# Sangluisme/PSgradientSDF

Hardware: AMD Instinct MI355X
Metric: Gauss-Newton iterations/sec (full PS sweep), 256^3 grid x 50 frames (higher is better)
Workload: dtype f32

## Files before the change

### __graft_entry__.py

```python
from __future__ import annotations

import ctypes
import os
import re
import subprocess
import sys

ROOT = os.path.dirname(os.path.abspath(__file__))
if ROOT not in sys.path:
    sys.path.insert(0, ROOT)


def _declared_symbols(header="psgsdf.h"):
    hdr = open(os.path.join(ROOT, "include", header)).read()
    hdr = re.sub(r"/\*.*?\*/", "", hdr, flags=re.S)
    return sorted(set(re.findall(r"\b(psgsdf_[a-z0-9_]+)\s*\(", hdr)) - {"psgsdf_iter_cb"})


def build() -> None:
    csrc = os.path.join(ROOT, "psgradientsdf_amd", "csrc")
    import glob, hashlib
    h = hashlib.sha256()
    for f in sorted(glob.glob(os.path.join(csrc, "*.hip")) + glob.glob(os.path.join(csrc, "*.h")) + glob.glob(os.path.join(ROOT, "psgradientsdf_amd", "host", "*.[ch]pp"))
                    + [os.path.join(csrc, "Makefile"), os.path.join(ROOT, "include", "psgsdf.h"), os.path.join(ROOT, "include", "psgsdf_render.h"),
                       os.path.join(ROOT, "include", "psgsdf_mesh.h"), os.path.join(ROOT, "include", "psgsdf_fit.h")]):
        h.update(os.path.relpath(f, ROOT).encode()); h.update(open(f, "rb").read())
    stamp = os.path.join(csrc, ".build_hash")
    clean = os.environ.get("PSGSDF_BUILD_CLEAN") == "1" or not os.path.exists(stamp) or open(stamp).read() != h.hexdigest() \
        or not os.path.exists(os.path.join(csrc, "libpsgsdf.so")) or not os.path.exists(os.path.join(csrc, "libpsgsdf_dev.so"))
    if clean:
        subprocess.check_call(["make", "-s", "-C", csrc, "clean"])
    import time
    t0 = time.time()
    subprocess.check_call(["make", "-s", "-j16", "-C", csrc])
    print(f"build: build_mode={'from_scratch' if clean else 'up_to_date_by_content_hash'} ({time.time() - t0:.0f} s, source hash {h.hexdigest()[:12]})")
    open(stamp, "w").write(h.hexdigest())
    subprocess.check_call(["make", "-s", "-C", os.path.join(ROOT, "oracle")])
    from psgradientsdf_amd import capi

    for path in (capi.ENGINE_LIB, capi.ENGINE_LIB_DEV):
        lib = ctypes.CDLL(path)
        missing = [s for s in _declared_symbols() + _declared_symbols("psgsdf_render.h") + _declared_symbols("psgsdf_mesh.h") + _declared_symbols("psgsdf_fit.h") if not hasattr(lib, s)]
        if missing:
            raise RuntimeError(f"{os.path.basename(path)} lacks {missing}")


def smoke() -> None:
    import numpy as np
    from psgradientsdf_amd import capi, synth
    from oracle import oracle

    sc = synth.make_scene(N=48, F=6, W=160, H=120, model="SH1")
    st = capi.default_settings(capi.SH1)
    eng = capi.load_engine(sc, sc.K, st, device=0)
    orc = oracle.Oracle(sc, sc.K, st)
    for api in (eng, orc):
        api.load_scene(sc)
        api.init_albedo()
        api.normalize_weights()
    assert eng.info().n_band == orc.info().n_band and eng.info().n_band > 1000
    re_, ro_ = eng.iterate(capi.ALL, 1)[0], orc.iterate(capi.ALL, 1)[0]
    de, do = eng.download_volume(), orc.download_volume()
    band = eng.download_band()
    vs = float(sc.voxel_size)
    err = np.abs(de["dist"][band] - do["dist"][band]).max() / vs
    print(f"smoke: band={len(band)} E_total engine={re_['e_total']:.6f} oracle={ro_['e_total']:.6f} max|d_gpu-d_cpu|/vs={err:.2e}")
    assert abs(re_["e_total"] - ro_["e_total"]) <= 1e-4 * abs(ro_["e_total"])
    assert err < 1e-3
    assert np.abs(eng.download_poses() - orc.download_poses()).max() < 1e-4


if __name__ == "__main__":
    build()
    if len(sys.argv) > 1 and sys.argv[1] == "smoke":
        smoke()
```

### psgradientsdf_amd/capi.py

```python
from __future__ import annotations

import ctypes as C
import os

import numpy as np

ALBEDO, LIGHT, DIST, POSE, ALL = 1, 2, 4, 8, 15
SH1, SH2, LED = 0, 1, 2
L2, CAUCHY, HUBER, TUKEY, TRUNC_L2 = 0, 1, 2, 3, 4
R_DEPTH, R_NORMAL, R_ALBEDO, R_SHADING, R_RENDERED, R_RESIDUAL, R_VOXEL = 1, 2, 4, 8, 16, 32, 64
R_ALL = 127
_R_PLANES = [("depth", R_DEPTH, 1), ("normal", R_NORMAL, 3), ("albedo", R_ALBEDO, 3), ("shading", R_SHADING, 1),
             ("rendered", R_RENDERED, 3), ("residual", R_RESIDUAL, 3), ("voxel", R_VOXEL, 1)]

_HERE = os.path.dirname(os.path.abspath(__file__))
ENGINE_LIB = os.environ.get("PSGSDF_ENGINE_LIB") or os.path.join(_HERE, "csrc", "libpsgsdf.so")
ENGINE_LIB_DEV = os.path.join(_HERE, "csrc", "libpsgsdf_dev.so")


class GridDesc(C.Structure):
    _fields_ = [("dim", C.c_int32 * 3), ("voxel_size", C.c_float), ("shift", C.c_float * 3), ("truncation", C.c_float)]


class Settings(C.Structure):
# ... 440 lines not shown

    def debug_overlap_probe(self, reps=10):
        out = (C.c_double * 4)()
        self._check(self._fn("debug_overlap_probe")(self.ctx, C.c_int(reps), out), "debug_overlap_probe")
        return list(out)

    def debug_normals_cache(self, width, height):
        out = np.empty((9, height, width), np.float32)
        self._check(self._fn("debug_normals_cache")(self.ctx, C.c_int(width), C.c_int(height), out.ctypes.data_as(C.c_void_p)), "debug_normals_cache")
        return out

    def comm_init_sockets(self, peer_fds, rank, n_ranks):
        fds = (C.c_int * n_ranks)(*[int(f) for f in peer_fds])
        self._check(self._fn("comm_init_sockets")(self.ctx, fds, C.c_int(rank), C.c_int(n_ranks)), "comm_init_sockets")

    def comm_allreduce_host(self, values):
        a = np.ascontiguousarray(values, np.float64).copy()
        self._check(self._fn("comm_allreduce_host")(self.ctx, a.ctypes.data_as(C.c_void_p), C.c_int(a.size)), "comm_allreduce_host")
        return a

    def comm_stats(self):
        n = C.c_int64()
        self._check(self._fn("comm_stats")(self.ctx, C.byref(n)), "comm_stats")
        return n.value

    def set_stream(self, stream_ptr):
        self._check(self._fn("set_stream")(self.ctx, C.c_void_p(stream_ptr)), "set_stream")

    def mg_info(self):
        out = (C.c_int32 * 12)()
        self._check(self._fn("mg_info")(self.ctx, out), "mg_info")
        return dict(zip(self._MG_INFO_NAMES, list(out)))

    _MG_INFO_NAMES = ["S", "rows", "row0", "row1", "halo", "F", "rank", "n_ranks", "need_lo", "need_hi", "z0", "z1"]

    def get_tuning(self):
        import json
        f = getattr(self._lib, self._p + "get_tuning"); f.restype = C.c_int
        n = f(self.ctx, None, C.c_size_t(0))
        if n < 0:
            self._check(n, "get_tuning")
        buf = C.create_string_buffer(n + 1)
        f(self.ctx, buf, C.c_size_t(n + 1))
        return json.loads(buf.value.decode())

    def set_profiling(self, on):
        self._check(self._fn("set_profiling")(self.ctx, C.c_int(1 if on else 0)), "set_profiling")

    def watch_kernel(self, name):
        self._check(self._fn("watch_kernel")(self.ctx, name.encode() if name else None), "watch_kernel")

    def reset_kernel_times(self):
        self._check(self._fn("reset_kernel_times")(self.ctx), "reset_kernel_times")

    def kernel_times(self):
        cap = 64
        names = (C.c_char_p * cap)(); ms = (C.c_double * cap)(); n = (C.c_int64 * cap)()
        f = getattr(self._lib, self._p + "kernel_times"); f.restype = C.c_int
        k = f(self.ctx, names, ms, n, C.c_int(cap))
        return {names[i].decode(): (ms[i], n[i]) for i in range(k)}

    def debug_dist_system(self, x=None):
        S = self.info().n_band
        diag = np.empty(S, np.float32); rhs = np.empty(S, np.float32)
        y = np.empty(S, np.float32) if x is not None else None
        xa = np.ascontiguousarray(x, np.float32) if x is not None else None
        self._check(self._fn("debug_dist_system")(self.ctx, diag.ctypes.data_as(C.c_void_p), rhs.ctypes.data_as(C.c_void_p),
                                                   xa.ctypes.data_as(C.c_void_p) if x is not None else None,
                                                   y.ctypes.data_as(C.c_void_p) if x is not None else None), "debug_dist_system")
        return diag, rhs, y

    def debug_time_pcg_pass(self, blocks=0, rows=2, ablate=0, reps=50, stamps=False):
        ms = C.c_double(0)
        st = np.zeros((max(blocks, 1), 8), np.int64) if stamps else None
        self._check(self._fn("debug_time_pcg_pass")(self.ctx, C.c_int(blocks), C.c_int(rows), C.c_int(ablate | (1024 if stamps else 0)), C.c_int(reps), C.byref(ms),
                                                     st.ctypes.data_as(C.c_void_p) if stamps else None), "debug_time_pcg_pass")
        return (ms.value, st) if stamps else ms.value

    def debug_time_pcg_solve(self, passes=16, reps=5):
        ms = C.c_double(0); shape = (C.c_int32 * 2)(); st = (C.c_double * 16)()
        self._check(self._fn("debug_time_pcg_solve")(self.ctx, C.c_int(passes), C.c_int(reps), C.byref(ms), shape, st), "debug_time_pcg_solve")
        return ms.value, (shape[0], shape[1]), [x for x in st]

    def debug_sync_stats(self):
        out = (C.c_int64 * 8)()
        self._check(self._fn("debug_sync_stats")(self.ctx, out), "debug_sync_stats")
        return dict(readbacks_checked=out[0], readbacks_late=out[1], persist_fallbacks=out[2] % 1000000, keyframes_compacted=out[2] // 1000000, speculative_starts=out[3] // 1000000, speculative_undos=out[3] % 1000000,
                    cross_rank_ready=out[4] % 10, halo_pushes=out[4] // 10, cross_rank_solves=out[5], cross_rank_mem_kind=out[6], probe_stale=out[7] // 1000000, probe_timeouts=out[7] % 1000000)

    def debug_rare_rows(self):
        r = C.c_int64(); w = C.c_int64()
        self._check(self._fn("debug_rare_rows")(self.ctx, C.byref(r), C.byref(w)), "debug_rare_rows")
        return r.value, w.value

    def debug_frame_system(self, block):
        i = self.info()
        if block == LIGHT:
            n = i.light_stride; nb = 1 if self._settings.model == LED else i.n_frames
        else:
            n = 6; nb = i.n_frames
        H = np.empty((nb, n, n), np.float64); b = np.empty((nb, n), np.float64)
        self._check(self._fn("debug_frame_system")(self.ctx, C.c_int(block), H.ctypes.data_as(C.c_void_p), b.ctypes.data_as(C.c_void_p)), "debug_frame_system")
        return H, b

    def set_frame_solver(self, mode):
        self._check(self._fn("set_frame_solver")(self.ctx, C.c_int(mode)), "set_frame_solver")

    def frame_solver_stats(self, block):
        it = C.c_int32(); err = C.c_double(); ok = C.c_int32(); ap = C.c_int32()
        self._check(self._fn("get_frame_solver_stats")(self.ctx, C.c_int(block), C.byref(it), C.byref(err), C.byref(ok), C.byref(ap)), "get_frame_solver_stats")
        return {"cg_iters": it.value, "cg_error": err.value, "cg_converged": ok.value, "applied": ap.value}

    def debug_frame_cg(self, H, b, max_it=0):
        H = np.ascontiguousarray(H, np.float32); b = np.ascontiguousarray(b, np.float32)
        nb, n = b.shape
        x = np.empty((nb, n), np.float32); it = C.c_int32(); err = C.c_double(); ok = C.c_int32()
        self._check(self._fn("debug_frame_cg")(self.ctx, C.c_int(nb), C.c_int(n), H.ctypes.data_as(C.c_void_p), b.ctypes.data_as(C.c_void_p), x.ctypes.data_as(C.c_void_p),
                                               C.c_int(max_it), C.byref(it), C.byref(err), C.byref(ok)), "debug_frame_cg")
        return x, it.value, err.value, bool(ok.value)

    def debug_albedo_system(self):
        S = self.info().n_band
        H = np.empty((S, 3), np.float32); b = np.empty((S, 3), np.float32)
        self._check(self._fn("debug_albedo_system")(self.ctx, H.ctypes.data_as(C.c_void_p), b.ctypes.data_as(C.c_void_p)), "debug_albedo_system")
        return H, b


class CommXfer(C.Structure):
    _fields_ = [("ptr_dev", C.c_void_p), ("bytes", C.c_size_t), ("peer", C.c_int)]


ALLREDUCE_FN = C.CFUNCTYPE(C.c_int, C.c_void_p, C.c_void_p, C.c_int, C.c_void_p)
SENDRECV_FN = C.CFUNCTYPE(C.c_int, C.c_void_p, C.POINTER(CommXfer), C.c_int, C.POINTER(CommXfer), C.c_int, C.c_void_p)


class CommOps(C.Structure):
    _fields_ = [("user", C.c_void_p), ("allreduce_f64", ALLREDUCE_FN), ("sendrecv", SENDRECV_FN)]


def comm_unique_id() -> bytes:
    buf = (C.c_uint8 * 128)()
    f = engine_lib().psgsdf_comm_unique_id; f.restype = C.c_int
    rc = f(buf)
    if rc != 0:
        raise PsgsdfError(f"psgsdf_comm_unique_id failed rc={rc} (librccl could not be loaded?)")
    return bytes(buf)


def grid_of(sc) -> GridDesc:
    g = GridDesc()
    g.dim[:] = [int(x) for x in sc.dim]
    g.voxel_size = float(sc.voxel_size)
    g.shift[:] = [float(x) for x in sc.shift]
    g.truncation = float(sc.truncation)
    return g


_engine_lib = {}


def engine_lib(dev: bool = False) -> C.CDLL:
    path = ENGINE_LIB_DEV if dev else ENGINE_LIB
    if path not in _engine_lib:
        if not os.path.exists(path):
            raise PsgsdfError(f"HIP engine {path} is missing: run `python -c 'import __graft_entry__ as g; g.build()'`")
        _engine_lib[path] = C.CDLL(path)
# ... 7 lines not shown
```

### psgradientsdf_amd/csrc/api.hip

```cpp
#include "engine_internal.h"

using namespace psge;

namespace psge {
int host_stage(psgsdf_ctx* c, size_t bytes, void** p) {
    if (c->pin_bytes < bytes) {
        HIPCHK(c, hipStreamSynchronize(c->stream));
        if (c->pin_stage) hipHostFree(c->pin_stage);
        c->pin_stage = nullptr; c->pin_bytes = 0;
        const size_t want = bytes + bytes / 4;
        HIPCHK(c, hipHostMalloc(&c->pin_stage, want, hipHostMallocDefault));
        c->pin_bytes = want;
    }
    *p = c->pin_stage;
    return 0;
}
}

extern "C" {

#ifdef PSGSDF_DEV
const char* psgsdf_version(void) { return "psgsdf-hip gfx950 r5 dev (fault-injection and ablation knobs compiled in: libpsgsdf_dev.so, tests and tools only)"; }
#else
const char* psgsdf_version(void) { return "psgsdf-hip gfx950 r5"; }
#endif

static const char* const kKnobs[] = {
    "PSGSDF_PCG_POLL", "PSGSDF_SPECULATE", "PSGSDF_FOLD_IN_NEXT", "PSGSDF_FUSE_ALBEDO", "PSGSDF_FUSE_PCG_INIT", "PSGSDF_PCG_PERSIST", "PSGSDF_PCG_XCD_LOCAL",
    "PSGSDF_PCG_FUSE_ASM", "PSGSDF_PCG_FUSE_APPLY", "PSGSDF_PCG_PIPELINE", "PSGSDF_PCG_TAGM", "PSGSDF_PCG_PREFETCH", "PSGSDF_PCG_COL16", "PSGSDF_PCG_ROWS", "PSGSDF_PCG_BLOCKS",
    "PSGSDF_FM_SOLVE", "PSGSDF_FRAME_SOLVE", "PSGSDF_FM_ROWS", "PSGSDF_IMG_COMPACT", "PSGSDF_XCD_MAP", "PSGSDF_XCD_STRIPE",
    "PSGSDF_XR", "PSGSDF_XF", "PSGSDF_XS", "PSGSDF_XH", "PSGSDF_XR_MEM", "PSGSDF_XWAIT_LOG2", "PSGSDF_SPECULATE_MR", "PSGSDF_CU_MASK",
    "PSGSDF_WAIT_TIMEOUT_S", "PSGSDF_DESTROY_TIMEOUT_S", "PSGSDF_SOLVE_DUMP"};
static const char* const kDevKnobs[] = {"PSGSDF_PCG_ABLATE", "PSGSDF_FAULT_SOLVE", "PSGSDF_FAULT_HALO", "PSGSDF_MBOX_CHECK"};
const char* psgsdf_last_error(const psgsdf_ctx* c) { return c ? c->err : "null context"; }

int psgsdf_create(const psgsdf_grid_desc* grid, const float K[9], const psgsdf_settings* settings, int device, psgsdf_ctx** out) {
    if (!grid || !K || !settings || !out) return PSGSDF_ERR_ARG;
    if (settings->model < 0 || settings->model > 2) return PSGSDF_ERR_ARG;
    int ndev = 0;
    if (hipGetDeviceCount(&ndev) != hipSuccess || ndev <= 0 || device < 0 || device >= ndev) return PSGSDF_ERR_DEVICE;
    if (hipSetDevice(device) != hipSuccess) return PSGSDF_ERR_DEVICE;
    psgsdf_ctx* c = new psgsdf_ctx();
    c->device = device;
    if (const char* e = getenv("PSGSDF_PCG_POLL")) c->pcg_poll = atoi(e) != 0;
    if (const char* e = getenv("PSGSDF_SPECULATE")) c->speculate = atoi(e) != 0;
    if (const char* e = getenv("PSGSDF_FOLD_IN_NEXT")) c->fold_in_next = atoi(e) != 0;
    if (const char* e = getenv("PSGSDF_FUSE_ALBEDO")) c->fuse_albedo = atoi(e) != 0;
    if (const char* e = getenv("PSGSDF_FUSE_PCG_INIT")) c->fuse_pcg_init = atoi(e) != 0;
    if (const char* e = getenv("PSGSDF_PCG_PERSIST")) c->pcg_persist = atoi(e) != 0;
    if (const char* e = getenv("PSGSDF_PCG_XCD_LOCAL")) c->pcg_xcd_local = atoi(e) != 0;
    if (const char* e = getenv("PSGSDF_AREG_DEVICE")) c->areg_device = atoi(e) != 0;
    if (const char* e = getenv("PSGSDF_PCG_FUSE_ASM")) c->pcg_fuse_asm = atoi(e) != 0;
    if (const char* e = getenv("PSGSDF_PCG_PIPELINE")) c->pcg_pipeline = atoi(e) != 0;
    if (const char* e = getenv("PSGSDF_PCG_TAGM")) { c->pcg_tagm = atoi(e) != 0; c->pcg_tagm_mr = atoi(e) >= 2; }
    if (const char* e = getenv("PSGSDF_PCG_PREFETCH")) c->pcg_prefetch = atoi(e) != 0;
    if (const char* e = getenv("PSGSDF_FM_SOLVE")) { c->fm_solve = atoi(e) != 0; c->fm_solve_led = atoi(e) == 1; }
    if (const char* e = getenv("PSGSDF_FRAME_SOLVE")) c->frame_solve = (!strcmp(e, "eigen") || !strcmp(e, "1")) ? 1 : 0;
    if (const char* e = getenv("PSGSDF_XF")) c->xf_enable = atoi(e) != 0;
    if (const char* e = getenv("PSGSDF_XS")) c->xs_enable = atoi(e) != 0;
    if (const char* e = getenv("PSGSDF_XH")) c->xh_enable = atoi(e) != 0;
    if (const char* e = getenv("PSGSDF_XWAIT_LOG2")) { const int l = atoi(e); if (l >= 8 && l <= 30) c->xwait_spins = 1 << l; }
    if (const char* e = getenv("PSGSDF_IMG_COMPACT")) c->img_compact = atoi(e) != 0;
    if (const char* e = getenv("PSGSDF_SPECULATE_MR")) c->speculate_mr = atoi(e) != 0;
    if (const char* e = getenv("PSGSDF_XCD_MAP")) c->xcd_map = atoi(e);
    if (const char* e = getenv("PSGSDF_XCD_STRIPE")) c->xcd_map = (c->xcd_map & 255) | (atoi(e) << 8);
#ifdef PSGSDF_DEV
    if (const char* e = getenv("PSGSDF_PCG_ABLATE")) c->pcg_ablate = atoi(e) & 7;
    if (const char* e = getenv("PSGSDF_MBOX_CHECK")) c->mbox_check = atoi(e) != 0;
    if (const char* e = getenv("PSGSDF_FAULT_SOLVE")) c->fault_solve = atoi(e);
    if (const char* e = getenv("PSGSDF_FAULT_HALO")) c->fault_halo = atoll(e);
#endif
    for (const char* k : kKnobs) if (const char* e = getenv(k)) c->tuning_env.emplace_back(k, e);
    for (const char* k : kDevKnobs) if (const char* e = getenv(k)) {
#ifdef PSGSDF_DEV
        c->tuning_env.emplace_back(k, e);
#else
        c->tuning_ignored.emplace_back(k, e);
#endif
    }
    if (const char* e = getenv("PSGSDF_PCG_FUSE_APPLY")) c->pcg_fuse_apply = atoi(e) != 0;
    if (hipDeviceGetAttribute(&c->num_cu, hipDeviceAttributeMultiprocessorCount, device) != hipSuccess) c->num_cu = 0;
    c->set = *settings; c->reg_n = settings->reg_weight_n; c->reg_l = settings->reg_weight_l; c->reg_r = settings->reg_weight_rho;
    GridP& g = c->grid;
    for (int a = 0; a < 3; ++a) { g.dim[a] = grid->dim[a]; c->shift[a] = grid->shift[a]; }
    g.nvox = (long long)g.dim[0] * g.dim[1] * g.dim[2]; g.koff = 0;
    for (int a = 0; a < 3; ++a) c->gdim[a] = g.dim[a];
    c->gnvox = g.nvox; c->z0 = c->zlo = 0; c->z1 = c->zhi = g.dim[2];
    g.vs = grid->voxel_size; g.vs_inv = 1.f / g.vs; g.T = grid->truncation;
    for (int a = 0; a < 3; ++a) g.origin[a] = c->shift[a] - (float)(0.5 * (double)g.vs) * (float)g.dim[a];
    c->cam.fx = K[0]; c->cam.fy = K[4]; c->cam.cx = K[2]; c->cam.cy = K[5];
    if (const char* e = getenv("PSGSDF_XR")) c->xr_enable = atoi(e) != 0;
    bool stream_ok;
    if (const char* e = getenv("PSGSDF_CU_MASK")) {
        int lo = 0, hi = 0;
        if (sscanf(e, "%d:%d", &lo, &hi) != 2 || lo < 0 || hi <= lo || hi > c->num_cu) { delete c; return PSGSDF_ERR_ARG; }
        std::vector<uint32_t> mask((size_t)(c->num_cu + 31) / 32, 0u);
        for (int i = lo; i < hi; ++i) mask[i / 32] |= 1u << (i % 32);
        stream_ok = hipExtStreamCreateWithCUMask(&c->stream, (uint32_t)mask.size(), mask.data()) == hipSuccess;
        c->cu_mask_lo = lo; c->cu_mask_hi = hi; c->num_cu = hi - lo;
    } else stream_ok = hipStreamCreate(&c->stream) == hipSuccess;
    bool ok = stream_ok
        && hipMalloc(&c->pcg_sc, sizeof(double) * (16 + 8 * (size_t)kPcgMaxBlocks)) == hipSuccess
        && hipMalloc(&c->pcg_part, sizeof(double) * 14 * kPcgMaxBlocks) == hipSuccess
        && hipMalloc(&c->pcg_gran, sizeof(double) * 2 * kSolveGranPlanes * kSolveMaxBlocksHost) == hipSuccess
        && hipMalloc(&c->mg_scal, sizeof(double) * kMgScal) == hipSuccess && hipMalloc(&c->mg_ext, sizeof(double) * 8) == hipSuccess
        && hipMalloc(&c->d_need, 2 * sizeof(int)) == hipSuccess
        && hipMalloc(&c->d_total, sizeof(int)) == hipSuccess
        && hipMalloc(&c->led_light, sizeof(float) * 3) == hipSuccess
        && hipMalloc(&c->fs_stats, sizeof(double) * 8) == hipSuccess && hipMemset(c->fs_stats, 0, sizeof(double) * 8) == hipSuccess
        && hipEventCreate(&c->ev0) == hipSuccess && hipEventCreate(&c->ev1) == hipSuccess;
    if (!ok) { delete c; return PSGSDF_ERR_DEVICE; }
    *out = c;
    return PSGSDF_OK;
}

void psgsdf_destroy(psgsdf_ctx* c) {
    if (!c) return;
    hipSetDevice(c->device);
    if (c->stream) hipStreamSynchronize(c->stream);
    double qt = 15.0; if (const char* e = getenv("PSGSDF_DESTROY_TIMEOUT_S")) qt = atof(e);
    if (xr_quiesce(c, qt)) {
        c->leak_exported = true;
        fprintf(stderr, "psgsdf: rank %d: a peer did not close its mappings of this rank's exchange memory within %.0f s (failed or still running?): that memory is leaked, not freed\n", c->rank, qt);
    }
    free_dense(c);
    hipFree(c->vis_seq); hipFree(c->frame_idx); hipFree(c->img); hipFree(c->img8); hipFree(c->frames); hipFree(c->frames_undo); hipFree(c->led_light); hipFree(c->fs_stats);
    hipFree(c->band_mem); if (!c->leak_exported) hipFree(c->rec_mem); hipFree(c->obs_mem); hipFree(c->stage);
    hipFree(c->ncache); hipFree(c->ntmp); hipFree(c->nout); hipFree(c->ndepth); hipFree(c->track_part); if (c->track_host) hipHostFree(c->track_host); hipFree(c->acc_frame); hipFree(c->frame_part); hipFree(c->frame_done); hipFree(c->part); hipFree(c->pcg_sc); hipFree(c->pcg_part); hipFree(c->pcg_gran); hipFree(c->d_total);
    for (void* p : c->xo_host) if (p) hipHostFree(p);
    if (c->pin_stage) hipHostFree(c->pin_stage);
    if (c->host_buf) hipHostFree(c->host_buf);
    if (c->mbox) hipHostFree(c->mbox);
    if (c->ev0) hipEventDestroy(c->ev0); if (c->ev1) hipEventDestroy(c->ev1);
    for (auto& pr : c->watch_pool) { hipEventDestroy(pr.first); hipEventDestroy(pr.second); }
    if (!c->leak_exported) { hipFree(c->xr); hipFree(c->hx_mem); }
    hipFree(c->xf_table); hipFree(c->vm_order);
    comm_destroy(c);
    hipFree(c->areg_mem); hipFree(c->mg_scal); hipFree(c->mg_ext); hipFree(c->mbox_shadow); hipFree(c->d_need);
    if (c->stream && c->own_stream) hipStreamDestroy(c->stream);
    delete c;
}

static double count_plane(const psgsdf_ctx* c, const float* d, const uint64_t* v, int wpv) {
    const long long plane = (long long)c->gdim[0] * c->gdim[1];
    const float lim = (float)(sqrt(3.0) * (double)c->grid.vs);
    long long m = 0;
    for (long long i = 0; i < plane; ++i) { if (!(fabsf(d[i]) <= lim)) continue; bool seen = false; for (int w = 0; w < wpv && !seen; ++w) seen = v[(size_t)i * wpv + w] != 0; m += seen; }
    return (double)m;
}
static int cut_slabs(psgsdf_ctx* c, std::vector<double>& cnt, int* z0, int* z1) {
    const int nz = c->gdim[2], n = c->n_ranks;
    if (nz < n) return fail(c, PSGSDF_ERR_UNSUPPORTED, "%d z-planes cannot be cut into %d slabs", nz, n);
    if (n > 1) {
        double* d_cnt = nullptr;
        HIPCHK(c, hipMalloc(&d_cnt, sizeof(double) * nz));
        int rc = 0;
        if (hipMemcpyAsync(d_cnt, cnt.data(), sizeof(double) * nz, hipMemcpyHostToDevice, c->stream) != hipSuccess) rc = fail(c, PSGSDF_ERR_DEVICE, "slab histogram upload");
        if (!rc) rc = comm_allreduce(c, d_cnt, nz);
        if (!rc && (hipMemcpyAsync(cnt.data(), d_cnt, sizeof(double) * nz, hipMemcpyDeviceToHost, c->stream) != hipSuccess || hipStreamSynchronize(c->stream) != hipSuccess)) rc = fail(c, PSGSDF_ERR_DEVICE, "slab histogram download");
        hipFree(d_cnt);
        if (rc) return rc;
    }
    double total = 0; for (double x : cnt) total += x;
    if (total <= 0) return fail(c, PSGSDF_ERR_UNSUPPORTED, "the volume has no band candidates to partition");
    std::vector<int> cut(n + 1, 0); cut[n] = nz;
    double run = 0; int r = 1;
    for (int k = 0; k < nz && r < n; ++k) { run += cnt[k]; while (r < n && run >= total * r / n) { cut[r] = k + 1; ++r; } }
    for (int q = 1; q < n; ++q) cut[q] = std::max(cut[q], cut[q - 1] + 1);
    for (int q = n - 1; q >= 1; --q) cut[q] = std::min(cut[q], cut[q + 1] - 1);
    *z0 = cut[c->rank]; *z1 = cut[c->rank + 1];
    return 0;
}
static int choose_slab(psgsdf_ctx* c, const float* dist, const uint64_t* vis_words, int wpv, int* z0, int* z1) {
    const int nz = c->gdim[2], n = c->n_ranks;
    const long long plane = (long long)c->gdim[0] * c->gdim[1];
    std::vector<double> cnt(nz, 0.0);
    for (int k = c->rank; k < nz; k += n) cnt[k] = count_plane(c, dist + (size_t)k * plane, vis_words + (size_t)k * plane * wpv, wpv);
    return cut_slabs(c, cnt, z0, z1);
}

static int upload_planes(psgsdf_ctx* c, int z0, int z1, size_t src_n, size_t src_off, const float* dist, const float* grad_xyz, const float* weight, const float* rgb, const uint64_t* vis_words, int words_per_voxel) {
    { int rc = set_local_grid(c, z0, z1); if (rc) return rc; }
    const long long n = c->grid.nvox;
    free_dense(c);
    if (c->vis_seq) { hipFree(c->vis_seq); c->vis_seq = nullptr; }
    int rc = alloc_dense(c, c->dense, n, 0, true); if (rc) return rc;
    HIPCHK(c, hipMalloc(&c->vis_seq, sizeof(uint64_t) * n * words_per_voxel));
    c->wpv_seq = words_per_voxel;
    HIPCHK(c, hipMemcpyAsync(c->dense.dist, dist + src_off, sizeof(float) * n, hipMemcpyHostToDevice, c->stream));
    for (int a = 0; a < 3; ++a) {
        HIPCHK(c, hipMemcpyAsync(c->dense.g[a], grad_xyz + (size_t)a * src_n + src_off, sizeof(float) * n, hipMemcpyHostToDevice, c->stream));
        HIPCHK(c, hipMemcpyAsync(c->dense.rho[a], rgb + (size_t)a * src_n + src_off, sizeof(float) * n, hipMemcpyHostToDevice, c->stream));
    }
    HIPCHK(c, hipMemcpyAsync(c->dense.weight, weight + src_off, sizeof(float) * n, hipMemcpyHostToDevice, c->stream));
    HIPCHK(c, hipMemcpyAsync(c->vis_seq, vis_words + src_off * words_per_voxel, sizeof(uint64_t) * n * words_per_voxel, hipMemcpyHostToDevice, c->stream));
    HIPCHK(c, hipStreamSynchronize(c->stream));
    c->have_volume = true; c->inited = false;
    return PSGSDF_OK;
}

int psgsdf_upload_volume(psgsdf_ctx* c, const float* dist, const float* grad_xyz, const float* weight, const float* rgb, const uint64_t* vis_words, int words_per_voxel) {
    if (!c || !dist || !grad_xyz || !weight || !rgb || !vis_words || words_per_voxel < 1) return fail(c, PSGSDF_ERR_ARG, "upload_volume: null argument");
    HIPCHK(c, hipSetDevice(c->device));
    int z0 = 0, z1 = c->gdim[2];
    if (c->n_ranks > 1) { int rc = choose_slab(c, dist, vis_words, words_per_voxel, &z0, &z1); if (rc) return rc; }
    const int zlo = std::max(0, z0 - 1);
    return upload_planes(c, z0, z1, (size_t)c->gnvox, (size_t)zlo * c->gdim[0] * c->gdim[1], dist, grad_xyz, weight, rgb, vis_words, words_per_voxel);
}

int psgsdf_slab_plane_count(psgsdf_ctx* c, const float* dist_plane, const uint64_t* vis_plane, int words_per_voxel, double* count) {
    if (!c || !dist_plane || !vis_plane || !count || words_per_voxel < 1) return fail(c, PSGSDF_ERR_ARG, "slab_plane_count: null argument");
// ... 432 lines not shown
```

### psgradientsdf_amd/csrc/api_debug.hip

```cpp
#include "engine_internal.h"

using namespace psge;

extern "C" {
int psgsdf_set_profiling(psgsdf_ctx* c, int enabled) { if (!c) return PSGSDF_ERR_ARG; c->profiling = enabled != 0; return PSGSDF_OK; }
int psgsdf_reset_kernel_times(psgsdf_ctx* c) { if (!c) return PSGSDF_ERR_ARG; c->ktimes.clear(); c->watch_used = 0; return PSGSDF_OK; }
int psgsdf_watch_kernel(psgsdf_ctx* c, const char* name) {
    if (!c) return PSGSDF_ERR_ARG;
    hipStreamSynchronize(c->stream);
    std::string w = name ? name : ""; int every = 1;
    const size_t sl = w.find('/');
    if (sl != std::string::npos) { every = std::max(1, atoi(w.c_str() + sl + 1)); w.resize(sl); }
    c->watch = w; c->watch_every = every; c->watch_seen = 0; c->watch_used = 0;
    return PSGSDF_OK;
}
int psgsdf_kernel_times(psgsdf_ctx* c, const char** names, double* ms, int64_t* launches, int cap) {
    if (!c) return 0;
    if (c->watch_used) {
        hipStreamSynchronize(c->stream);
        KTime& k = c->ktimes[c->watch];
        for (size_t i = 0; i < c->watch_used; ++i) { float t = 0; if (hipEventElapsedTime(&t, c->watch_pool[i].first, c->watch_pool[i].second) == hipSuccess) { k.ms += t; k.n += 1; } }
        c->watch_used = 0;
    }
    int n = 0;
    for (auto& kv : c->ktimes) { if (n >= cap) break; names[n] = kv.first.c_str(); ms[n] = kv.second.ms; launches[n] = kv.second.n; ++n; }
    return n;
}

int psgsdf_debug_dist_system(psgsdf_ctx* c, float* diag, float* rhs, const float* x, float* y) {
    if (!c || !c->inited) return fail(c, PSGSDF_ERR_STATE, "init first");
    HIPCHK(c, hipSetDevice(c->device));
    SweepArgs a = make_args(c, c->reg_l != 0.f);
    launch_sweep_dist(a, c->stream);
    launch_assemble(a, c->stream);
    const int S = c->band.S;
    if (diag) HIPCHK(c, hipMemcpyAsync(diag, c->band.H, sizeof(float) * S, hipMemcpyDeviceToHost, c->stream));
    if (rhs) HIPCHK(c, hipMemcpyAsync(rhs, c->band.rhs, sizeof(float) * S, hipMemcpyDeviceToHost, c->stream));
    if (x && y) {
        HIPCHK(c, hipMemcpyAsync(c->band.x, x, sizeof(float) * S, hipMemcpyHostToDevice, c->stream));
        launch_matvec(a, c->band.x, c->band.t, c->stream);
        HIPCHK(c, hipMemcpyAsync(y, c->band.t, sizeof(float) * S, hipMemcpyDeviceToHost, c->stream));
    }
    HIPCHK(c, hipStreamSynchronize(c->stream));
    return PSGSDF_OK;
}

int psgsdf_debug_time_pcg_pass(psgsdf_ctx* c, int blocks, int rows, int ablate, int reps, double* avg_ms, long long* stamps) {
    if (!c || !c->inited || !avg_ms) return fail(c, PSGSDF_ERR_STATE, "init first");
    HIPCHK(c, hipSetDevice(c->device));
    SweepArgs a = make_args(c, c->reg_l != 0.f);
    launch_sweep_dist(a, c->stream);
    launch_assemble(a, c->stream);
    int G, rdef; cgf_shape(band_blocks(c), &G, &rdef);
    if (blocks > 0) G = std::min(blocks, kCgfMaxBlocks);
    if (rows <= 0) rows = rdef;
    launch_cgf_init(a, c->pcg_sc, c->pcg_part, G, c->stream);
    hipEvent_t e0, e1; HIPCHK(c, hipEventCreate(&e0)); HIPCHK(c, hipEventCreate(&e1));
    for (int q = 0; q < 3; ++q) launch_cgf_pass(a, c->pcg_sc, c->pcg_part, G, rows, q, 1 << 30, c->mbox_dev, c->stream, ablate | 16);
    HIPCHK(c, hipEventRecord(e0, c->stream));
    for (int q = 0; q < reps; ++q) launch_cgf_pass(a, c->pcg_sc, c->pcg_part, G, rows, 3 + q, 1 << 30, c->mbox_dev, c->stream, ablate | 16);
    HIPCHK(c, hipEventRecord(e1, c->stream));
    HIPCHK(c, hipStreamSynchronize(c->stream));
    float ms = 0; HIPCHK(c, hipEventElapsedTime(&ms, e0, e1));
    hipEventDestroy(e0); hipEventDestroy(e1);
    *avg_ms = (double)ms / reps;
    if (stamps) {
        HIPCHK(c, hipMemcpy(stamps, c->pcg_sc + 16, sizeof(long long) * 8 * G, hipMemcpyDeviceToHost));
    }
    return PSGSDF_OK;
}

int psgsdf_debug_time_pcg_solve(psgsdf_ctx* c, int passes, int reps, double* ms_per_launch, int32_t* shape, double* stamps ) {
    if (!c || !c->inited || !ms_per_launch || !shape || (passes < 1 && passes != -7) || reps < 1) return fail(c, PSGSDF_ERR_STATE, "init first");
    HIPCHK(c, hipSetDevice(c->device));
    int G = 0, rows = 0;
    if (!cgf_solve_shape(c, &G, &rows)) return fail(c, PSGSDF_ERR_UNSUPPORTED, "the persistent solve does not apply to this context");
    shape[0] = G; shape[1] = rows;
    SweepArgs a = make_args(c, c->reg_l != 0.f);
    a.pcg_fuse_init = 1; a.pcg_init_blocks = band_blocks(c); a.pcg_gran = c->pcg_gran; a.pcg_gran_n = 2 * kSolveGranPlanes * kSolveMaxBlocksHost; a.pcg_asm = c->pcg_fuse_asm ? 1 : 0;
    hipEvent_t e0, e1; HIPCHK(c, hipEventCreate(&e0)); HIPCHK(c, hipEventCreate(&e1));
    float total = 0;
    for (int r = 0; r < reps + 1; ++r) {
        launch_sweep_dist(a, c->stream);
// ... 76 lines not shown
    if (!c) return PSGSDF_ERR_ARG;
    if (mode != 0 && mode != 1) return fail(c, PSGSDF_ERR_ARG, "frame solver mode %d (0 = LDL^T per frame, 1 = the reference's global float Jacobi-PCG)", mode);
    c->frame_solve = mode;
    return PSGSDF_OK;
}
int psgsdf_get_frame_solver_stats(psgsdf_ctx* c, int block, int32_t* iterations, double* error, int32_t* converged, int32_t* applied) {
    if (!c) return PSGSDF_ERR_ARG;
    if (block != PSGSDF_LIGHT && block != PSGSDF_POSE) return fail(c, PSGSDF_ERR_ARG, "block must be LIGHT or POSE");
    HIPCHK(c, hipSetDevice(c->device));
    const int kind = block == PSGSDF_POSE ? 1 : 0;
    psgsdf_step_stats st; memset(&st, 0, sizeof(st));
    if (int rc = read_frame_solver_stats(c, kind, &st)) return rc;
    if (iterations) *iterations = st.cg_iters;
    if (error) *error = st.cg_error;
    if (converged) *converged = st.cg_converged;
    if (applied) *applied = st.applied;
    return PSGSDF_OK;
}
int psgsdf_debug_frame_cg(psgsdf_ctx* c, int nb, int n, const float* H, const float* b, float* x, int max_it, int32_t* iterations, double* error, int32_t* converged) {
    if (!c || !H || !b || !x || nb <= 0) return fail(c, PSGSDF_ERR_ARG, "null argument");
    if ((n != 3 && n != 4 && n != 6 && n != 9) || (long long)nb * n > 2048) return fail(c, PSGSDF_ERR_UNSUPPORTED, "block size %d x %d blocks", n, nb);
    HIPCHK(c, hipSetDevice(c->device));
    float *dH = nullptr, *db = nullptr, *dx = nullptr; double* ds = nullptr;
    const size_t nH = (size_t)nb * n * n, nv = (size_t)nb * n;
    int rc = PSGSDF_OK;
    if (hipMalloc(&dH, sizeof(float) * nH) != hipSuccess || hipMalloc(&db, sizeof(float) * nv) != hipSuccess || hipMalloc(&dx, sizeof(float) * nv) != hipSuccess || hipMalloc(&ds, sizeof(double) * 4) != hipSuccess)
        rc = fail(c, PSGSDF_ERR_DEVICE, "out of device memory");
    double st[4] = {0, 0, 0, 0};
    if (!rc && (hipMemcpy(dH, H, sizeof(float) * nH, hipMemcpyHostToDevice) != hipSuccess || hipMemcpy(db, b, sizeof(float) * nv, hipMemcpyHostToDevice) != hipSuccess)) rc = fail(c, PSGSDF_ERR_DEVICE, "upload failed");
    if (!rc && launch_frames_eigen_raw(nb, n, dH, db, dx, ds, max_it, c->stream)) rc = fail(c, PSGSDF_ERR_UNSUPPORTED, "shape");
    if (!rc && (hipStreamSynchronize(c->stream) != hipSuccess || hipMemcpy(x, dx, sizeof(float) * nv, hipMemcpyDeviceToHost) != hipSuccess || hipMemcpy(st, ds, sizeof(st), hipMemcpyDeviceToHost) != hipSuccess))
        rc = fail(c, PSGSDF_ERR_DEVICE, "%s", hipGetErrorString(hipGetLastError()));
    hipFree(dH); hipFree(db); hipFree(dx); hipFree(ds);
    if (rc) return rc;
    if (iterations) *iterations = (int32_t)st[0];
    if (error) *error = st[1];
    if (converged) *converged = (int32_t)st[2];
    return PSGSDF_OK;
}
int psgsdf_debug_frame_system(psgsdf_ctx* c, int block, double* H, double* b) {
    if (!c || !c->inited || !H || !b) return fail(c, PSGSDF_ERR_STATE, "init first");
    HIPCHK(c, hipSetDevice(c->device));
    SweepArgs a = make_args(c, 0);
    const bool led = c->set.model == PSGSDF_LED;
    int n, nb, nh;
    int launched = 0;
    if (block == PSGSDF_LIGHT) { launched = launch_sweep_light(a, c->stream); n = led ? 3 : (c->set.model == PSGSDF_SH2 ? 9 : 4); nb = led ? 1 : c->F; nh = led ? 3 : n * (n + 1) / 2; }
    else if (block == PSGSDF_POSE) { launched = launch_sweep_pose(a, c->stream); n = 6; nb = c->F; nh = 21; }
    else return fail(c, PSGSDF_ERR_ARG, "block must be LIGHT or POSE");
    if (!launched) HIPCHK(c, hipMemsetAsync(c->acc_frame, 0, sizeof(double) * c->acc_frame_n, c->stream));
    std::vector<double> acc(c->acc_frame_n);
    HIPCHK(c, hipMemcpyAsync(acc.data(), c->acc_frame, sizeof(double) * c->acc_frame_n, hipMemcpyDeviceToHost, c->stream));
    HIPCHK(c, hipStreamSynchronize(c->stream));
    if (led && block == PSGSDF_LIGHT) {
        for (int i = 0; i < 9; ++i) H[i] = 0;
        for (int i = 0; i < 3; ++i) { b[i] = 0; for (int f = 0; f < c->F; ++f) { H[i * 3 + i] += acc[(size_t)f * kFrameRow + i]; b[i] += acc[(size_t)f * kFrameRow + 3 + i]; } }
        return PSGSDF_OK;
    }
    for (int k = 0; k < nb; ++k) {
        const double* A = acc.data() + (size_t)k * kFrameRow;
        double* Hk = H + (size_t)k * n * n; double* bk = b + (size_t)k * n;
        for (int i = 0; i < n * n; ++i) Hk[i] = 0;
        int q = 0;
        for (int i = 0; i < n; ++i) for (int j = i; j < n; ++j) { Hk[i * n + j] = A[q]; Hk[j * n + i] = A[q]; ++q; }
        for (int i = 0; i < n; ++i) bk[i] = A[nh + i];
    }
    return PSGSDF_OK;
}

int psgsdf_debug_albedo_system(psgsdf_ctx* c, float* H, float* b) {
    if (!c || !c->inited || !H || !b) return fail(c, PSGSDF_ERR_STATE, "init first");
    HIPCHK(c, hipSetDevice(c->device));
    SweepArgs a = make_args(c, 0);
    launch_sweep_albedo(a, c->stream);
    const int S = c->band.S, Sp = c->band.Spad;
    std::vector<float> h(3 * (size_t)Sp), bb(3 * (size_t)Sp);
    HIPCHK(c, hipMemcpyAsync(h.data(), c->band.aH, sizeof(float) * 3 * Sp, hipMemcpyDeviceToHost, c->stream));
    HIPCHK(c, hipMemcpyAsync(bb.data(), c->band.ab, sizeof(float) * 3 * Sp, hipMemcpyDeviceToHost, c->stream));
    HIPCHK(c, hipStreamSynchronize(c->stream));
    for (int j = 0; j < S; ++j) for (int ch = 0; ch < 3; ++ch) { H[3 * j + ch] = h[(size_t)ch * Sp + j]; b[3 * j + ch] = bb[(size_t)ch * Sp + j]; }
    return PSGSDF_OK;
}

int psgsdf_debug_sync_stats(psgsdf_ctx* c, int64_t out[8]) {
    if (!c || !out) return PSGSDF_ERR_ARG;
    out[0] = c->mbox_checked; out[1] = c->mbox_late; out[2] = c->persist_fallbacks + (c->img_compacted ? 1000000LL : 0); out[3] = c->spec_windows * 1000000LL + c->spec_undos;
    out[4] = (c->xr_ready ? 1 : 0) + 10 * c->n_halo_pushes; out[5] = c->xr_solves; out[6] = c->xr_mem_kind; out[7] = c->xr_probe_stale * 1000000LL + c->xr_probe_timeouts;
    return PSGSDF_OK;
}

int psgsdf_get_tuning(psgsdf_ctx* c, char* json, size_t cap) {
    if (!c) return PSGSDF_ERR_ARG;
    std::string o = "{\"build\": \"";
    o += psgsdf_version(); o += "\", \"env\": {";
    auto esc = [](const std::string& v) { std::string r; for (char ch : v) { if (ch == '"' || ch == '\\') r += '\\'; if ((unsigned char)ch >= 0x20) r += ch; } return r; };
    bool first = true;
    for (auto& kv : c->tuning_env) { o += (first ? "\"" : ", \"") + kv.first + "\": \"" + esc(kv.second) + "\""; first = false; }
    o += "}, \"ignored_dev_only\": {"; first = true;
    for (auto& kv : c->tuning_ignored) { o += (first ? "\"" : ", \"") + kv.first + "\": \"" + esc(kv.second) + "\""; first = false; }
    o += "}, \"effective\": {";
    char buf[1024];
    snprintf(buf, sizeof(buf), "\"pcg_poll\": %d, \"speculate\": %d, \"speculate_mr\": %d, \"fold_in_next\": %d, \"fuse_albedo\": %d, \"fuse_pcg_init\": %d, \"pcg_persist\": %d, \"pcg_pipeline\": %d, \"pcg_tagm\": %d, "
             "\"pcg_prefetch\": %d, \"pcg_fuse_asm\": %d, \"pcg_fuse_apply\": %d, \"pcg_xcd_local\": %d, \"fm_solve\": %d, \"fm_solve_led\": %d, \"frame_solve\": \"%s\", \"img_compact\": %d, \"xcd_map\": %d, "
             "\"xr\": %d, \"xf\": %d, \"xs\": %d, \"xh\": %d, \"xr_mem_kind\": %d, \"xwait_log2\": %d, \"cu_mask\": [%d, %d], \"mbox_check\": %d, \"pcg_ablate\": %d, \"fault_solve\": %d, \"fault_halo\": %lld",
             (int)c->pcg_poll, (int)c->speculate, (int)c->speculate_mr, (int)c->fold_in_next, (int)c->fuse_albedo, (int)c->fuse_pcg_init, (int)c->pcg_persist, (int)c->pcg_pipeline, (c->pcg_pipeline && c->pcg_tagm) ? (c->n_ranks > 1 ? (c->pcg_tagm_mr ? 2 : 0) : 1) : 0,
             (int)c->pcg_prefetch, (int)c->pcg_fuse_asm, (int)c->pcg_fuse_apply, (int)c->pcg_xcd_local, (int)c->fm_solve, (int)c->fm_solve_led, c->frame_solve == 1 ? "eigen" : "ldlt", (int)c->img_compact, c->xcd_map,
             (int)c->xr_enable, (int)c->xf_enable, (int)c->xs_enable, (int)c->xh_enable, c->xr_mem_kind, (int)lround(log2((double)c->xwait_spins)), c->cu_mask_lo, c->cu_mask_hi,
             (int)c->mbox_check, c->pcg_ablate, c->fault_solve, c->fault_halo);
    o += buf; o += "}";
    if (c->n_ranks > 1) {
        snprintf(buf, sizeof(buf), ", \"xr_probe\": {\"rank\": %d, \"n_ranks\": %d, \"kind_chosen\": %d, \"stale_mappings\": %lld, \"fine_grained\": {\"tried\": %lld, \"stale_records_from_lower\": %lld, \"expired_waits_lower\": %lld, \"expired_waits_upper\": %lld}, "
                 "\"uncached\": {\"tried\": %lld, \"stale_records_from_lower\": %lld, \"expired_waits_lower\": %lld, \"expired_waits_upper\": %lld}}",
                 c->rank, c->n_ranks, c->xr_mem_kind, c->xr_stale_maps, c->xr_probe_local[1][3], c->xr_probe_local[1][0], c->xr_probe_local[1][1], c->xr_probe_local[1][2],
                 c->xr_probe_local[2][3], c->xr_probe_local[2][0], c->xr_probe_local[2][1], c->xr_probe_local[2][2]);
        o += buf;
    }
    o += "}";
    if (json && cap) { const size_t n = std::min(cap - 1, o.size()); memcpy(json, o.data(), n); json[n] = 0; }
    return (int)o.size();
}

}
```

### psgradientsdf_amd/csrc/engine.h

```cpp
#pragma once
#include <hip/hip_runtime.h>
#include <stdint.h>

namespace psg {

constexpr int kBlock = 256;
constexpr int kMaxFramesLds = 640;
constexpr int kNQ = 19;
constexpr int kNQCommon = 13;
constexpr int kMaxBasis = 9;

struct FrameP {
    float R[9];
    float t[3];
    float l[9];
    float pad[3];
};

struct Cam { float fx, fy, cx, cy; int W, H; };

struct GridP {
    int dim[3];
    long long nvox;
    float vs, vs_inv;
// ... 22 lines not shown
    float4* vp[3];
    float* aH; float* ab;
    float* blk;
    float* H;
    int* hx;
    float* rhs; float* x; float* t;
    float4* rec[2];
    int* obs_ptr;
    int* obs_rows;
    int obs_max;
    long long obs_ptr_total;
};

struct Accum {
    double* frame;
    double* part;
    int PB;
    double* fpart;
    int fcap;
    int* fdone;
};
constexpr int kFrameRow = 64;
constexpr int kPcgMaxBlocks = 2048;
constexpr int kCgfMaxBlocks = 768;

enum { SC_ENERGY = 0, SC_NOBS = 1, SC_EN = 2, SC_EL = 3, SC_ACCEPT = 4, SC_AUX0 = 5, SC_AUX1 = 6, SC_AUX2 = 7, SC_COUNT = 8 };

struct AlbedoReg {
    int* anb;
    int* back;
    float* anrho;
    float* J;
    float* res;
    float* rhs; float* diag; float* diag0; float* x; float* r; float* p; float* q; float* t;
    double* cgs;
    float weight;
};

struct XfTable;
struct FoldReq { int n; int id[4]; int nblk; double* out; unsigned long long key; const XfTable* xf; long long xf_epoch; };

struct ImgSrc {
    const float* f32;
    const unsigned* u8; float scale;
    bool idx32;
};

struct SweepArgs {
    Band b;
    const FrameP* frames;
    ImgSrc im;
    int F;
    Cam cam;
    GridP grid;
    Robust rob;
    Accum acc;
    int model;
    int quirks;
    float reg_n, reg_l;
    int normal_reg, laplacian_reg;
    float damping;
    int row0, row1;
    FoldReq fold;
    AlbedoReg ar;
    double* pcg_part; double* pcg_fs;
    int pcg_asm;
    unsigned pcg_epoch;
    int pcg_pipe;
    int pcg_xcd_local;
    int pcg_apply;
    double* pcg_gran; int pcg_gran_n;
    int pcg_fuse_init;
    int pcg_init_blocks;
    int fuse_apply;
    const int* vm_order;
    float* fm_led_light;
    const XfTable* xf;
    long long xf_epoch;
    int xcd_map;
    int fm_solve;
    FrameP* fm_frames; float* fm_undo; double* fm_e_out; unsigned long long fm_e_key;
    const double* gate;
    const double* ext;
};

constexpr int kXrMaxRanks = 32;
constexpr int kXrPeerTags = 64;
constexpr int kXrRankGran = 0, kXrPtag = 2 * 8 * kXrMaxRanks, kXrAbort = kXrPtag + 2 * 3 * kXrPeerTags, kXrDoubles = kXrAbort + 8;
constexpr int kXrLate = kXrAbort + 1;
constexpr int kXrNonce = kXrAbort + 7;
struct XrArgs {
    int rank, n_ranks;
    double* region[kXrMaxRanks];
    float4* lo_rec[2]; float4* hi_rec[2];
    float4* lo_base[2];
    int give_lo, give_hi;
    int wait_lo, wait_hi;
    int need_lo, need_hi;
    unsigned epoch;
};
struct XfTable {
    int n_ranks, rank, F, spin_max;
    long long pay, flg;
    long long spay, sflg;
    double* region[32];
};
constexpr int kHxWords = 16;
constexpr unsigned kXrEpochMask = 0x3fffu;

constexpr int kTryPackFlags = 2048;
void launch_normals_cache(int W, int H, int r, double fx_inv, double fy_inv, double cx, double cy, double* work , float* out , hipStream_t s);
void launch_try_pack_f32(const float* rgb, unsigned* rgba, size_t npix, size_t stride, float scale, int* fail , hipStream_t s);
void launch_pack_rgb8(const uint8_t* rgb, unsigned* rgba, size_t npix, hipStream_t s);
void launch_select_vis(const uint64_t* vis_seq, int wpv_seq, uint64_t* vis_key, int KW, const int* frame_idx, int F, long long nvox, hipStream_t s);
void launch_band_flags(const float* dist, const uint64_t* vis_key, int KW, float vs, long long nvox, int* flags, hipStream_t s);
void launch_band_scan(int* flags_inout_rowof, long long nvox, int* block_sums, int* d_total, hipStream_t s);
struct DenseView { float* dist; float* g[3]; float* weight; float* rho[3]; uint64_t* vis; int KW; int* row_of; };
void launch_band_fill(const DenseView& d, const GridP& grid, Band b, int* d_reach, hipStream_t s);
void launch_band_scatter(const DenseView& d, Band b, hipStream_t s);
void launch_derive(const SweepArgs& a, int update_grad, hipStream_t s);
constexpr int kObsChunk = 2048;
void launch_obs_count(const Band& b, int F, int row0, int row1, int* counts, hipStream_t s);
void launch_block_work(const Band& b, int row0, int row1, int* work, hipStream_t s);
void launch_obs_fill(const Band& b, int F, int row0, int row1, const int* offsets, hipStream_t s);
void launch_lower_bound(const int* lin, int S, int target, int* out, hipStream_t s);
struct SlotList { int n; int id[8]; };
void launch_sum_parts(const double* part, int PB, int nblk, const SlotList& slots, double* out, unsigned long long key, hipStream_t s, const XfTable* xf = nullptr, long long xf_epoch = 0);
void launch_frame_cols(const double* frame, int F, int col, double* out, unsigned long long key, hipStream_t s);
void launch_zero_f64(double* p, int n, hipStream_t s);
struct CopySegs { int n; unsigned off[16]; unsigned len[16]; unsigned long long key[16]; };
void launch_copy_segs(const double* src, double* dst, const CopySegs& segs, hipStream_t s);
void launch_marker(double* p, double v, hipStream_t s);
void launch_init_albedo(const SweepArgs& a, hipStream_t s);
void launch_led_light_init(const SweepArgs& a, hipStream_t s);
void launch_energy(const SweepArgs& a, hipStream_t s);
void launch_sweep_albedo(const SweepArgs& a, hipStream_t s);
void launch_apply_albedo(const SweepArgs& a, hipStream_t s);
void launch_restore_albedo(const SweepArgs& a, hipStream_t s);
int launch_sweep_light(const SweepArgs& a, hipStream_t s);
int launch_sweep_pose(const SweepArgs& a, hipStream_t s);
void launch_solve_light(const SweepArgs& a, FrameP* frames, float* led_light, double* e_out, unsigned long long e_key, float* undo, hipStream_t s);
void launch_restore_light(int F, FrameP* frames, float* led_light, const float* undo, hipStream_t s);
void launch_solve_pose(const SweepArgs& a, FrameP* frames, double* e_out, unsigned long long e_key, hipStream_t s);
bool frames_eigen_fits(int model, int F);
void launch_frames_eigen_light(const SweepArgs& a, FrameP* frames, float* led_light, double* e_out, unsigned long long e_key, float* undo, double* stats, hipStream_t s);
void launch_frames_eigen_pose(const SweepArgs& a, FrameP* frames, double* e_out, unsigned long long e_key, double* stats, hipStream_t s);
int launch_frames_eigen_raw(int nb, int n, const float* H, const float* b, float* x, double* stats, int max_it, hipStream_t s);
void launch_sweep_dist(const SweepArgs& a, hipStream_t s);
void launch_assemble(const SweepArgs& a, hipStream_t s);
void launch_cgf_init(const SweepArgs& a, double* fs, double* part, int G, hipStream_t s);
void launch_cgf_pass(const SweepArgs& a, double* fs, double* part, int G, int rows, int k, int kmax, double* mb, hipStream_t s, int ablate = 0);
void launch_cgf_sum(double* part, int G, int k, double* out, hipStream_t s);
constexpr int kSolveGranPlanes = 8;
constexpr int kSolveThreadsHost = 512, kSolveMaxBlocksHost = 256, kSolveMaxRowsHost = 4, kSolveMbSlots = 24;
int cgf_solve_max_blocks(int rows);
void launch_cgf_solve(const SweepArgs& a, double* fs, double* gran, int G, int rows_per_wg, int kmax, double* mb, unsigned long long mb_key, int force_passes, hipStream_t s, const XrArgs* xr = nullptr);
void launch_areg_tables(const DenseView& d, const GridP& g, const SweepArgs& a, hipStream_t s);
void launch_areg_build(const SweepArgs& a, hipStream_t s);
void launch_areg_system(const SweepArgs& a, hipStream_t s);
void launch_areg_jx(const SweepArgs& a, const float* p, float* t, hipStream_t s);
void launch_areg_jt(const SweepArgs& a, const float* p, const float* t, float* q, hipStream_t s);
void launch_areg_cg_init(const SweepArgs& a, hipStream_t s);
void launch_areg_cg_iteration(const SweepArgs& a, int i, int nblk, float thr, hipStream_t s);
void launch_areg_cg_update(const SweepArgs& a, float alpha, hipStream_t s);
void launch_areg_cg_dir(const SweepArgs& a, float beta, hipStream_t s);
void launch_apply_albedo_delta(const SweepArgs& a, const float* delta, hipStream_t s);
void launch_matvec(const SweepArgs& a, const float* x, float* y, hipStream_t s);
void launch_apply_dist(const SweepArgs& a, hipStream_t s);
void launch_upsample(const DenseView& src, const DenseView& dst, const GridP& g_old, hipStream_t s);
void launch_fill_f32(float* p, float v, long long n, hipStream_t s);
void launch_normals(const float* depth, const float* cache, int W, int H, int r, double* tmp, float* out, hipStream_t s);
void launch_track(const DenseView& d, const GridP& g, const Cam& cam, const FrameP& fp, const float* depth, float z_min, float z_max, double* part, int nblk, int gdimz, int zown0, int zown1, hipStream_t s);
void launch_integrate(const DenseView& d, uint64_t* vis_seq, int wpv_seq, const GridP& g, const Cam& cam, const FrameP& fp,
                      const float* rgb, const float* depth, const float* normals, int counter, float z_min, float z_max, hipStream_t s);

constexpr int kRenderBrick = 8;
constexpr int kRenderTile = 8;
constexpr int kRenderStats = 9;
enum { RP_DEPTH = 0, RP_NORMAL, RP_ALBEDO, RP_SHADING, RP_RENDERED, RP_RESIDUAL, RP_VOXEL, RP_COUNT };
enum { RF_DEPTH = 0, RF_NORMAL = 1, RF_ALBEDO = 4, RF_SHADING = 7, RF_RENDERED = 8, RF_VOXEL = 11, RF_OFF_BAND = 12, RF_COUNT = 13 };
struct RenderArgs {
    DenseView d;
    const float4* vp[3];
    GridP grid;
    const FrameP* frames;
    ImgSrc im; int img_w, img_h;
    Robust rob;
    const unsigned char* bricks;
    const int* bbox;
    int nb[3];
    Cam cam;
    int frame;
    int light_frame;
    FrameP pose;
    int tiles_x, tiles_y;
    float* planes[RP_COUNT];
    double* part;
    int zr[2];
    int slab;
    int f0;
    double* mask;
    unsigned char* mine;
    double* rec;
    long long rec_px;
    int rf[RF_COUNT];
    int n_rf;
};
void launch_render_bricks(const DenseView& d, const GridP& g, float thr, int z0, int z1, unsigned char* bricks, int* bbox, double* marks, hipStream_t s);
void launch_render_box(const double* marks, const int* nb, unsigned char* bricks, int* bbox, hipStream_t s);
void launch_render(const RenderArgs& a, int model, hipStream_t s);
void launch_render_report(const RenderArgs& a, int model, int F, hipStream_t s);
void launch_render_fold(const double* part, int tiles, int F, double* out , hipStream_t s);
void launch_render_ranks(const RenderArgs& a, int model, bool report, int chunk, hipStream_t s);
void launch_render_keep(const RenderArgs& a, hipStream_t s);
void launch_render_composite(const RenderArgs& a, bool report, int chunk, hipStream_t s);

struct WMeshGrid {
    const float* dist; const float* weight; const float* g[3]; const float* rho[3];
    const float* hg[3]; const float* hrho[3];
    int nx, ny, zlo, zh;
    int lo[3], d[3];
    int zc0;
    long long nown;
    float voxel[3], origin[3];
};
void launch_wmesh_mark(const WMeshGrid& g, long long ncell, int* cnt, int* flag, hipStream_t s);
void launch_wmesh_or(int* dst, const int* src, long long n, hipStream_t s);
void launch_wmesh_faces(const WMeshGrid& g, long long ncell, const int* offs, int n_faces, const int* num, int first, const int* num_up, int first_up, int* faces, hipStream_t s);
void launch_wmesh_verts(const WMeshGrid& g, const int* num, int n_verts, float* xyz, float* nrm, unsigned char* rgb, hipStream_t s);

void launch_band_fit(const SweepArgs& a, int* n_obs, double* loss, float* sum_r2, hipStream_t s);
void launch_wmesh_fit(const WMeshGrid& g, const int* num, int n_verts, const int* row_of, int row0, int row1, const int* n_obs, const double* loss, const float* sum_r2,
                      int* v_n, float* v_rms, float* v_loss, hipStream_t s);

enum { MC_FIRST = 0, MC_VERTS, MC_FACES, MC_EDGES, MC_BOUNDARY, MC_NONMANIFOLD, MC_AREA, kMcompStats = 8 };
void launch_mcomp_init(int* parent, int nv, hipStream_t s);
void launch_mcomp_hook(const int* faces, int nf, int* parent, hipStream_t s);
void launch_mcomp_flatten(int* parent, int nv, int* flag, hipStream_t s);
// ... 11 lines not shown
```

### psgradientsdf_amd/csrc/engine.hip

```cpp
#include "engine_internal.h"
#include <chrono>
#include <sched.h>

namespace psge {

int wait_mapped(psgsdf_ctx* c, const std::function<bool()>& ready, const char* what) {
    using clk = std::chrono::steady_clock;
    static const double limit_s = [] { const char* e = getenv("PSGSDF_WAIT_TIMEOUT_S"); double v = e ? atof(e) : 0.0; return v > 0.0 ? v : 120.0; }();
    clk::time_point t0{}, next_query{};
    bool timing = false;
    for (unsigned spin = 1;; ++spin) {
        if (ready()) return 0;
        if (spin & 0x3ffu) continue;
        const clk::time_point now = clk::now();
        if (!timing) { timing = true; t0 = now; next_query = now + std::chrono::milliseconds(20); continue; }
        if (now - t0 > std::chrono::milliseconds(2)) sched_yield();
        if (now < next_query) continue;
        next_query = now + std::chrono::milliseconds(20);
        const hipError_t q = hipStreamQuery(c->stream);
        if (q == hipSuccess) return ready() ? 0 : 1;
        if (q != hipErrorNotReady) return fail(c, PSGSDF_ERR_DEVICE, "%s: stream error while waiting: %s", what, hipGetErrorString(q));
        if (std::chrono::duration<double>(now - t0).count() > limit_s)
            return fail(c, PSGSDF_ERR_DEVICE, "%s: nothing published within %.0f s (PSGSDF_WAIT_TIMEOUT_S)", what, limit_s);
    }
}

int fail(psgsdf_ctx* c, int code, const char* fmt, ...) {
    if (c) { va_list ap; va_start(ap, fmt); vsnprintf(c->err, sizeof(c->err), fmt, ap); va_end(ap); }
    return code;
}
SweepArgs make_args(psgsdf_ctx* c, int laplacian_reg) {
    SweepArgs a{};
    a.b = c->band; a.frames = c->frames; a.F = c->F; a.cam = c->cam; a.grid = c->grid;
    a.im.f32 = c->img; a.im.u8 = c->img8; a.im.scale = c->img_scale;
    a.im.idx32 = (size_t)c->F * c->cam.W * c->cam.H * 12 < ((size_t)1 << 32) && (size_t)c->F * c->cam.H < ((size_t)1 << 24) && 3 * (size_t)c->cam.W < ((size_t)1 << 24);
    a.rob.loss = c->set.loss; a.rob.lambda = c->set.lambda; a.rob.lambda_sq = c->set.lambda * c->set.lambda; a.rob.inv_lambda = 1.0f / c->set.lambda;
    a.acc.frame = c->acc_frame; a.acc.part = c->part; a.acc.PB = c->PB;
    a.acc.fpart = c->frame_part; a.acc.fcap = c->frame_cap; a.acc.fdone = c->frame_done;
    a.fold.n = 0; a.gate = nullptr; a.fuse_apply = 0;
    a.xcd_map = c->xcd_map; a.xf = nullptr; a.xf_epoch = 0; a.fm_led_light = nullptr; a.vm_order = c->vm_order;
    a.fm_solve = 0; a.fm_frames = nullptr; a.fm_undo = nullptr; a.fm_e_out = nullptr; a.fm_e_key = 0;
    a.pcg_part = c->pcg_part; a.pcg_fs = c->pcg_sc; a.pcg_fuse_init = 0; a.pcg_init_blocks = 0; a.pcg_gran = nullptr; a.pcg_gran_n = 0; a.pcg_asm = 0; a.pcg_epoch = 0; a.pcg_pipe = c->pcg_pipeline ? (c->pcg_tagm ? (c->n_ranks <= 1 ? 2 : (c->pcg_tagm_mr ? 3 : 1)) : 1) : 0; a.pcg_apply = 0; a.pcg_xcd_local = (c->pcg_xcd_local ? 1 : 0) | (c->pcg_prefetch ? 2 : 0) | (c->pcg_ablate << 3);
    a.ar = c->ar; a.ar.weight = c->reg_r;
    a.model = c->set.model; a.quirks = c->set.ref_quirks;
    a.reg_n = c->reg_n; a.reg_l = c->reg_l;
    a.normal_reg = c->reg_n != 0.0f; a.laplacian_reg = laplacian_reg;
    a.damping = c->set.damping;
    a.row0 = c->row0; a.row1 = c->row1;
    a.ext = nullptr;
    return a;
}

int read_parts(psgsdf_ctx* c, const int* slots, int n, double* out) {
    int rc = read_parts_deferred(c, slots, n, [out, n](const double* v) { for (int i = 0; i < n; ++i) out[i] = v[i]; });
    return rc ? rc : flush(c);
}
int read_frame_energy(psgsdf_ctx* c, int col_e, double* E, double* nobs) {
    int rc = read_frame_energy_deferred(c, col_e, [E, nobs](double e, double n) { *E = e; *nobs = n; });
    return rc ? rc : flush(c);
}
bool readback_landed(const Deferred& d) {
    const volatile double* v = d.src;
    for (int i = 0; i < d.n; ++i) if ((dbits(v[i]) ^ dbits(v[d.n + i])) != d.key + (unsigned long long)i) return false;
    return true;
}
int deliver_first(psgsdf_ctx* c, size_t count, bool told_landed) {
    count = std::min(count, c->deferred.size());
    for (size_t e = 0; e < count; ++e) {
        Deferred& d = c->deferred[e];
        if (d.key && c->mbox_check) {
            c->mbox_checked++;
            if (!readback_landed(d)) {
                if (told_landed) c->mbox_late++;
                const Deferred* dp = &d;
                const int w = wait_mapped(c, [dp] { return readback_landed(*dp); }, "read-back");
                if (w < 0) return w;
                if (w == 1) { HIPCHK(c, hipStreamSynchronize(c->stream)); if (!readback_landed(d)) return fail(c, PSGSDF_ERR_DEVICE, "a scalar read-back never arrived (the kernel that owed it did not run)"); }
            }
        }
        d.consume(d.src);
    }
    c->deferred.erase(c->deferred.begin(), c->deferred.begin() + (long)count);
    if (c->deferred.empty()) c->mbox_used = 0;
    if (c->mbox && c->mbox_n && ((volatile double*)c->mbox)[c->mbox_n + 1] != 0.0) {
        const double ep = ((volatile double*)c->mbox)[c->mbox_n + 1];
        ((volatile double*)c->mbox)[c->mbox_n + 1] = 0.0;
        return fail(c, PSGSDF_ERR_DEVICE, "rank %d of %d: halo pull %.0f gave up -- a neighbour's halo rows never arrived within the bounded wait (2^%d polls); the halo rows were filled with NaN", c->rank, c->n_ranks, ep, (int)log2((double)c->xwait_spins));
    }
    if (c->xf_timeout) {
        c->xf_timeout = false;
        double late[4] = {0, 0, 0, 0};
        if (c->xr) { (void)hipStreamSynchronize(c->stream); if (hipMemcpy(late, c->xr + kXrLate, sizeof(late), hipMemcpyDeviceToHost) != hipSuccess) (void)hipGetLastError(); }
        if (late[0] == 0 && late[1] == 0 && late[2] == 0)
            return fail(c, PSGSDF_ERR_DEVICE, "rank %d of %d: NaN came back from an exchange between the ranks' kernels, and no bounded wait of this rank expired: a peer handed on NaN (its wait expired, or the state itself is NaN)", c->rank, c->n_ranks);
        return fail(c, PSGSDF_ERR_DEVICE, "rank %d of %d: NaN came back from an exchange between the ranks' kernels -- a peer's contribution never arrived within the bounded wait (2^%d polls): frame rows of exchange %.0f (missing: rank %d's row of frame %d), scalar fold %.0f, halo pull %.0f (0 = not that one)",
                    c->rank, c->n_ranks, (int)log2((double)c->xwait_spins), late[0], (int)late[3] / 1000, (int)late[3] % 1000, late[1], late[2]);
    }
    return 0;
}
int deliver(psgsdf_ctx* c) { return deliver_first(c, c->deferred.size(), true); }
int mbox_reserve(psgsdf_ctx* c, int n, size_t* off, unsigned long long* key) {
    if (c->mbox_used + 2 * (size_t)n > c->mbox_n) { int rc = flush(c); if (rc) return rc; }
    *off = c->mbox_used; c->mbox_used += 2 * (size_t)n;
    *key = (++c->mbox_serial << 8) | 0x80u;
    return 0;
}
int flush(psgsdf_ctx* c) {
    materialize_fold(c);
    { int rc = mg_commit(c); if (rc) return rc; }
    bool synced = false;
    if (c->pcg_poll && !c->profiling && c->mbox && c->mbox_check && !c->deferred.empty() && c->deferred.back().key) {
        const Deferred& d = c->deferred.back();
        const volatile double* v = d.src; const int n = d.n; const unsigned long long key = d.key;
        const int w = wait_mapped(c, [v, n, key] { for (int i = 0; i < n; ++i) if ((dbits(v[i]) ^ dbits(v[n + i])) != key + (unsigned long long)i) return false; return true; }, "flush");
        if (w < 0) return w;
        synced = w == 0;
    } else if (c->pcg_poll && !c->profiling && c->mbox) {
        const double seq = (c->flush_seq += 1.0);
        launch_marker(c->mbox_dev + c->mbox_n, seq, c->stream);
        volatile double* m = c->mbox + c->mbox_n;
        const int w = wait_mapped(c, [m, seq] { return *m == seq; }, "flush");
        if (w < 0) return w;
        synced = w == 0;
    }
    if (!synced) HIPCHK(c, hipStreamSynchronize(c->stream));
// ... 193 lines not shown
        AlbedoReg& ar = c->ar;
        ar.anb = (int*)tk(3); ar.back = (int*)tk(1); ar.anrho = (float*)tk(9); ar.J = (float*)tk(12); ar.res = (float*)tk(3);
        ar.rhs = (float*)tk(3); ar.diag = (float*)tk(3); ar.diag0 = (float*)tk(3); ar.x = (float*)tk(3); ar.r = (float*)tk(3); ar.p = (float*)tk(3); ar.q = (float*)tk(3); ar.t = (float*)tk(3); ar.cgs = (double*)tk(1);
        SweepArgs at{}; at.b = b; at.ar = ar;
        launch_areg_tables(c->dense, c->grid, at, c->stream);
        if (int hrc = comm_halo(c, ar.back, 1, 1)) return hrc;
    }
    {
        const int nch = (c->row1 - c->row0 + kObsChunk - 1) / kObsChunk, F = c->F;
        if (c->obs_mem) { hipFree(c->obs_mem); c->obs_mem = nullptr; }
        b.obs_ptr = nullptr; b.obs_rows = nullptr; b.obs_max = 0; b.obs_ptr_total = 0;
        if (nch > 0 && F > 0) {
            int* d_counts = nullptr;
            HIPCHK(c, hipMalloc(&d_counts, sizeof(int) * (size_t)nch * F));
            launch_obs_count(b, F, c->row0, c->row1, d_counts, c->stream);
            std::vector<int> cnt((size_t)nch * F), off((size_t)nch * F), ptr(F + 1);
            HIPCHK(c, hipMemcpyAsync(cnt.data(), d_counts, sizeof(int) * cnt.size(), hipMemcpyDeviceToHost, c->stream));
            HIPCHK(c, hipStreamSynchronize(c->stream));
            int run = 0, mx = 0;
            for (int f = 0; f < F; ++f) { ptr[f] = run; for (int k = 0; k < nch; ++k) { off[(size_t)f * nch + k] = run; run += cnt[(size_t)f * nch + k]; } mx = std::max(mx, run - ptr[f]); }
            ptr[F] = run;
            HIPCHK(c, hipMalloc(&c->obs_mem, sizeof(int) * ((size_t)run + F + 2)));
            b.obs_ptr = (int*)c->obs_mem; b.obs_rows = b.obs_ptr + (F + 1); b.obs_max = mx; b.obs_ptr_total = run;
            HIPCHK(c, hipMemcpyAsync(b.obs_ptr, ptr.data(), sizeof(int) * (F + 1), hipMemcpyHostToDevice, c->stream));
            HIPCHK(c, hipMemcpyAsync(d_counts, off.data(), sizeof(int) * off.size(), hipMemcpyHostToDevice, c->stream));
            launch_obs_fill(b, F, c->row0, c->row1, d_counts, c->stream);
            HIPCHK(c, hipStreamSynchronize(c->stream));
            hipFree(d_counts);
        }
    }
    {
        if (c->vm_order) { hipFree(c->vm_order); c->vm_order = nullptr; }
        const int nb = (c->row1 - c->row0 + kBlock - 1) / kBlock;
        if (nb > 1) {
            int* d_work = nullptr;
            HIPCHK(c, hipMalloc(&d_work, sizeof(int) * nb));
            launch_block_work(b, c->row0, c->row1, d_work, c->stream);
            std::vector<int> work(nb), order(nb);
            HIPCHK(c, hipMemcpyAsync(work.data(), d_work, sizeof(int) * nb, hipMemcpyDeviceToHost, c->stream));
            HIPCHK(c, hipStreamSynchronize(c->stream));
            for (int i = 0; i < nb; ++i) order[i] = i;
            std::stable_sort(order.begin(), order.end(), [&](int x, int y) { return work[x] > work[y]; });
            HIPCHK(c, hipMalloc(&c->vm_order, sizeof(int) * nb));
            HIPCHK(c, hipMemcpyAsync(c->vm_order, order.data(), sizeof(int) * nb, hipMemcpyHostToDevice, c->stream));
            HIPCHK(c, hipStreamSynchronize(c->stream));
            hipFree(d_work);
        }
    }
    c->any_empty_slab = false;
    if (c->n_ranks > 1 && c->comm) {
        std::vector<double> e(1, (c->row1 <= c->row0 || b.obs_max <= 0) ? 1.0 : 0.0);
        if (int hrc = host_allreduce(c, e, "empty slabs")) return hrc;
        c->any_empty_slab = e[0] != 0.0;
    }
    {
        if (c->frame_part) { hipFree(c->frame_part); c->frame_part = nullptr; }
        if (c->frame_done) { hipFree(c->frame_done); c->frame_done = nullptr; }
        c->frame_cap = (b.obs_max + kBlock * 4 - 1) / (kBlock * 4) + 1;
        const int F = std::max(c->F, 1);
        HIPCHK(c, hipMalloc(&c->frame_part, sizeof(double) * (size_t)F * c->frame_cap * kFrameRow));
        HIPCHK(c, hipMalloc(&c->frame_done, sizeof(int) * (F + 1)));
        HIPCHK(c, hipMemsetAsync(c->frame_done, 0, sizeof(int) * (F + 1), c->stream));
    }
    if (c->part) { hipFree(c->part); c->part = nullptr; }
    c->PB = Spad / kBlock + 1;
    HIPCHK(c, hipMalloc(&c->part, sizeof(double) * SC_COUNT * c->PB));
    HIPCHK(c, hipMemsetAsync(c->part, 0, sizeof(double) * SC_COUNT * c->PB, c->stream));
    {
        const size_t need = 4096;
        if (need > c->mbox_alloc) {
            if (c->mbox) hipHostFree(c->mbox);
            c->mbox = nullptr; c->mbox_n = 0; c->mbox_alloc = 0;
            HIPCHK(c, hipHostMalloc(&c->mbox, sizeof(double) * need, hipHostMallocMapped));
            HIPCHK(c, hipHostGetDevicePointer((void**)&c->mbox_dev, c->mbox, 0));
            c->mbox_alloc = need; c->mbox_n = need - 2;
            memset(c->mbox, 0, sizeof(double) * need); c->flush_seq = 0;
        }
        if (slab_mode(c) && !c->mbox_shadow) {
            HIPCHK(c, hipMalloc(&c->mbox_shadow, sizeof(double) * c->mbox_alloc));
            HIPCHK(c, hipMemsetAsync(c->mbox_shadow, 0, sizeof(double) * c->mbox_alloc, c->stream));
        }
        c->mbox_used = 0; c->deferred.clear(); c->mg_segs.clear();
    }
    return ensure_host_buf(c, (size_t)SC_COUNT * c->PB + (size_t)c->F * kFrameRow + 4096 + 64);
}

int derive(psgsdf_ctx* c, int update_grad) {
    SweepArgs a = make_args(c, 0);
    timed(c, "derive", [&] { launch_derive(a, update_grad, c->stream); });
    const int slots[2] = {SC_EN, SC_EL}; double s[2];
    int rc = read_parts(c, slots, 2, s); if (rc) return rc;
    c->en_sum = s[0]; c->el_sum = s[1];
    return 0;
}


int ps_energy(psgsdf_ctx* c, double* E, int64_t* nobs) {
    SweepArgs a = make_args(c, 0);
    take_fold(c, a, (1u << SC_ENERGY) | (1u << SC_NOBS) | (1u << SC_AUX0) | (1u << SC_AUX1) | (1u << SC_AUX2));
    timed(c, "energy", [&] { launch_energy(a, c->stream); });
    const int slots[2] = {SC_ENERGY, SC_NOBS}; double s[2];
    int rc = read_parts(c, slots, 2, s); if (rc) return rc;
    *E = band_mean(c, s[0]); if (nobs) *nobs = (int64_t)s[1];
    return 0;
}

}
```

### psgradientsdf_amd/csrc/engine_internal.h

```cpp
#pragma once
#include "engine.h"
#include "../../include/psgsdf.h"

#include <math.h>
#include <float.h>
#include <stdarg.h>
#include <stdio.h>
#include <stdlib.h>
#include <string.h>
#include <algorithm>
#include <functional>
#include <memory>
#include <map>
#include <string>
#include <vector>

namespace psge {
constexpr int kMgScal = 96;
struct KTime { double ms = 0; int64_t n = 0; };
struct Comm;
struct MgSeg { unsigned off, n; unsigned long long key; };
struct Deferred { const double* src; int n; unsigned long long key; std::function<void(const double*)> consume; };
enum XoSlot {
    XO_MESH_XYZ, XO_MESH_RGB,
    XO_PC_XYZN, XO_PC_RGB,
    XO_SDF,
    XO_IMESH_XYZ, XO_IMESH_NORMALS, XO_IMESH_RGB, XO_IMESH_FACES,
    XO_VERTEX_COMPONENT, XO_COMPONENTS,
    XO_LOD_VERTEX_MAP,
    XO_FIT_NOBS, XO_FIT_LOSS, XO_FIT_R2,
    XO_VFIT_NOBS, XO_VFIT_RMS, XO_VFIT_LOSS,
    XO_COUNT
};
}
using psge::KTime;
using namespace psg;

struct psgsdf_ctx {
    int device = 0;
    hipStream_t stream = nullptr;
    psgsdf_settings set{};
    float reg_n = 0, reg_l = 0;
    GridP grid{};
    int gdim[3]{}; long long gnvox = 0;
    int z0 = 0, z1 = 0;
    int zlo = 0, zhi = 0;
    long long S_global = 0;
    float shift[3]{};
    Cam cam{};
    DenseView dense{};
    uint64_t* vis_seq = nullptr; int wpv_seq = 0;
    int* block_sums = nullptr; int* d_total = nullptr;
    bool have_volume = false;
    int F = 0;
    int* frame_idx = nullptr;
    float* img = nullptr;
    FrameP* frames = nullptr;
    std::vector<FrameP> frames_h;
    float* led_light = nullptr;
    bool have_frames = false;
    void* band_mem = nullptr; size_t band_bytes = 0;
    void* rec_mem = nullptr;
    void* obs_mem = nullptr;
    float* stage = nullptr; size_t stage_px = 0;
    void* pin_stage = nullptr; size_t pin_bytes = 0;
    float* ncache = nullptr; double* ntmp = nullptr; float* nout = nullptr; float* ndepth = nullptr; int ncache_w = 0, ncache_h = 0;
    double* track_part = nullptr; double* track_host = nullptr;
    Band band{};
    bool inited = false;
    double* acc_frame = nullptr; size_t acc_frame_n = 0;
    double* frame_part = nullptr; int frame_cap = 0;
    int* frame_done = nullptr;
    double* part = nullptr; int PB = 0;
    double* pcg_sc = nullptr; int pcg_cap = 4096;
    double* pcg_part = nullptr;
    double* pcg_gran = nullptr;
    bool pcg_fuse_asm = true;
    unsigned pcg_solve_serial = 0;
    bool pcg_tagm_mr = true;
    bool pcg_tagm = true;
    int pcg_ablate = 0;
    bool pcg_prefetch = true;
    bool pcg_pipeline = true;
    bool pcg_fuse_apply = true;
    bool pcg_xcd_local = true;
    bool pcg_persist = true;
    bool persist_off = false;
    int num_cu = 0;
    int last_cg_iters = 0;
    bool want_counts = true;
    double* host_buf = nullptr; size_t host_buf_n = 0;
    double* mbox = nullptr; double* mbox_dev = nullptr; size_t mbox_n = 0, mbox_used = 0;
    size_t mbox_alloc = 0; double flush_seq = 0;
    std::vector<psge::Deferred> deferred;
    unsigned long long mbox_serial = 0;
    bool mbox_check = true;
    psgsdf_iter_cb observer = nullptr; void* observer_user = nullptr;
    int on_iter_period = 1;
    bool speculate = true;
    bool spec_undo = false, spec_albedo_saved = false, spec_light_saved = false;
    FrameP* frames_undo = nullptr;
    long long spec_windows = 0, spec_undos = 0;
    int fault_solve = 0, solves_seen = 0;
    long long persist_fallbacks = 0;
    long long mbox_checked = 0, mbox_late = 0;
    double en_sum = 0, el_sum = 0;
    int rank = 0, n_ranks = 1;
    int row0 = 0, row1 = 0, halo = 0;
    psge::Comm* comm = nullptr;
    bool xr_enable = true;
    bool xr_ready = false; long long xr_solves = 0;
    double* xr = nullptr;
    int xr_mem_kind = -1;
    long long xr_probe_stale = 0, xr_probe_timeouts = 0;
    long long xr_probe_local[3][4] = {{0, 0, 0, 0}, {0, 0, 0, 0}, {0, 0, 0, 0}};
    bool xr_mapped = false;
    std::shared_ptr<void> comm_keep;
    unsigned long long xr_openers = 0;
    long long xr_serial = 0, xr_closed_off = 0;
    void* xo_host[psge::XO_COUNT] = {}; size_t xo_bytes[psge::XO_COUNT] = {};
    long long xr_stale_maps = 0;
    bool leak_exported = false;
    std::vector<double*> xr_peer;
    void* band_peer[2] = {nullptr, nullptr};
    std::vector<void*> xr_opened;
    XrArgs xr_args{};
    int cu_mask_lo = -1, cu_mask_hi = -1;
    double* mg_scal = nullptr;
    double* mg_ext = nullptr;
    double* mbox_shadow = nullptr;
    std::vector<psge::MgSeg> mg_segs;
    int give[2] = {0, 0};
    bool halo_active = false;
    long long n_collectives = 0;
    float reg_r = 0.f;
    void* areg_mem = nullptr; AlbedoReg ar{};
    bool areg_device = true; int areg_last_iters = 0;
    double er_sum = 0;
    FoldReq pending_fold{};
    bool fuse_pcg_init = true;
    bool fuse_albedo = true;
    bool fold_in_next = true;
    int xwait_spins = 1 << 24;
    long long fault_halo = 0;
    bool xh_enable = true;
    void* hx_mem = nullptr;
    char* hx_peer[2] = {nullptr, nullptr};
    size_t hx_peer_par[2] = {0, 0}, hx_peer_off[2] = {0, 0}, hx_par = 0;
    long long hx_flag_off = 0, hx_epoch = 0, n_halo_pushes = 0;
    bool hx_ready = false;
    bool xs_enable = true;
    long long xs_epoch = 0;
    bool xf_enable = true;
    XfTable* xf_table = nullptr;
    long long xf_epoch = 0;
    size_t xr_doubles = 0;
    bool any_empty_slab = false;
    bool xf_timeout = false;
    bool img_compact = true;
    bool img_compacted = false;
    bool speculate_mr = true;
    int* vm_order = nullptr;
    int xcd_map = 163;
    bool fm_solve = true;
    bool fm_solve_led = true;
// ... 31 lines not shown
    DevMem& operator=(const DevMem&) = delete;
    ~DevMem() { if (c) hipStreamSynchronize(c->stream); for (void* q : p) hipFree(q); }
    template <class T> bool get(T** out, size_t count) {
        void* q = nullptr;
        const bool ok = hipMalloc(&q, std::max<size_t>(8, sizeof(T) * count)) == hipSuccess;
        if (ok) p.push_back(q);
        *out = (T*)q;
        return ok;
    }
private:
    psgsdf_ctx* c; std::vector<void*> p;
};

template <class Fn> void timed(psgsdf_ctx* c, const char* name, Fn&& fn) {
    if (!c->profiling) {
        if (!c->watch.empty() && c->watch == name && (c->watch_seen++ % c->watch_every) == 0) {
            if (c->watch_used == c->watch_pool.size()) {
                hipEvent_t a, b; hipEventCreate(&a); hipEventCreate(&b); c->watch_pool.emplace_back(a, b);
            }
            auto& pr = c->watch_pool[c->watch_used++];
            hipEventRecord(pr.first, c->stream);
            fn();
            hipEventRecord(pr.second, c->stream);
            return;
        }
        fn(); return;
    }
    hipEventRecord(c->ev0, c->stream);
    fn();
    hipEventRecord(c->ev1, c->stream);
    hipEventSynchronize(c->ev1);
    float ms = 0; hipEventElapsedTime(&ms, c->ev0, c->ev1);
    KTime& k = c->ktimes[name]; k.ms += ms; k.n += 1;
}

int wait_mapped(psgsdf_ctx* c, const std::function<bool()>& ready, const char* what);

int comm_unique_id(uint8_t id[128]);
int comm_create_rccl(psgsdf_ctx* c, const uint8_t id[128], int rank, int n);
int comm_create_ext(psgsdf_ctx* c, const psgsdf_comm_ops* ops, int rank, int n);
void comm_destroy(psgsdf_ctx* c);
int comm_allreduce(psgsdf_ctx* c, double* buf, int n);
int comm_halo(psgsdf_ctx* c, void* base, int planes, int width);
int comm_xfer(psgsdf_ctx* c, const std::vector<psgsdf_comm_xfer>& sends, const std::vector<psgsdf_comm_xfer>& recvs);
int host_allreduce(psgsdf_ctx* c, std::vector<double>& buf, const char* what);
int xr_setup(psgsdf_ctx* c, const std::vector<double>& part_info);
void xr_release(psgsdf_ctx* c);
int xr_quiesce(psgsdf_ctx* c, double timeout_s);
int xr_probe(psgsdf_ctx* c);
int xr_alloc(psgsdf_ctx* c, void** p, size_t bytes, bool polled);
int mg_commit(psgsdf_ctx* c);
int set_local_grid(psgsdf_ctx* c, int z0, int z1);

int host_stage(psgsdf_ctx* c, size_t bytes, void** p);
int frontend_normals_dev(psgsdf_ctx* c, const float* d_depth, int width, int height, float* d_normals);
SweepArgs make_args(psgsdf_ctx* c, int laplacian_reg);
inline bool slab_mode(const psgsdf_ctx* c) { return c->comm != nullptr || c->n_ranks > 1; }
inline bool xs_active(const psgsdf_ctx* c) { return c->n_ranks > 1 && c->xs_enable && c->xr_ready && c->xf_table != nullptr; }
inline int band_blocks(const psgsdf_ctx* c) { return (c->row1 - c->row0 + kBlock - 1) / kBlock; }
inline double band_mean(const psgsdf_ctx* c, double sum) { return c->S_global ? sum / (double)c->S_global : 0.0; }
inline float total_energy(const psgsdf_ctx* c, float E, float E_n, float E_l, float E_r = 0.f) { return E + c->reg_n * E_n + c->reg_l * E_l + c->reg_r * E_r; }
int flush(psgsdf_ctx* c);
int mbox_reserve(psgsdf_ctx* c, int n, size_t* off, unsigned long long* key);
int deliver(psgsdf_ctx* c);
int deliver_first(psgsdf_ctx* c, size_t count, bool told_landed);
bool readback_landed(const psge::Deferred& d);
int read_parts(psgsdf_ctx* c, const int* slots, int n, double* out);
int read_frame_energy(psgsdf_ctx* c, int col_e, double* E, double* nobs);
int read_parts_deferred(psgsdf_ctx* c, const int* slots, int n, std::function<void(const double*)> consume);
int read_frame_energy_deferred(psgsdf_ctx* c, int col_e, std::function<void(double, double)> consume);
int reserve_frame_energy_deferred(psgsdf_ctx* c, std::function<void(double, double)> consume, double** dev_slot, unsigned long long* key);
void materialize_fold(psgsdf_ctx* c);
void fold_by_kernel(psgsdf_ctx* c, FoldReq& f);
void take_fold(psgsdf_ctx* c, SweepArgs& a, unsigned writes);
int ensure_host_buf(psgsdf_ctx* c, size_t n);
void free_dense(psgsdf_ctx* c);
int alloc_dense(psgsdf_ctx* c, DenseView& d, long long nvox, int KW, bool with_rowof);
int build_band(psgsdf_ctx* c);
int derive(psgsdf_ctx* c, int update_grad);
int ps_energy(psgsdf_ctx* c, double* E, int64_t* nobs);

struct LoopState { float E, E_n, E_l, E_prev; int laplacian_reg; float E_r; };
void cgf_shape(int nblk, int* G, int* rows);
bool cgf_solve_shape(psgsdf_ctx* c, int* G, int* rows, bool any_ranks = false);
int pcg_solve(psgsdf_ctx* c, SweepArgs& a, int* iters_out, int* success_out, double* err_out,
              const std::function<void(const double*)>& tail = nullptr, bool gate_on_converged = true, bool* tail_ran = nullptr);
int albedo_reg_energy(psgsdf_ctx* c, double* Er);
int albedo_reg_solve(psgsdf_ctx* c, const SweepArgs& a, int* iters_out, int* ok_out, double* err_out);
int step_begin(psgsdf_ctx* c, int block, int laplacian_reg, psgsdf_step_stats* st, std::function<void(double, double)> deferred_consumer = nullptr, bool may_apply = true);
int step_finish(psgsdf_ctx* c, int block, int laplacian_reg, psgsdf_step_stats* st, bool defer_reg_sums = false);
int do_step(psgsdf_ctx* c, int block, int laplacian_reg, psgsdf_step_stats* st);
int read_frame_solver_stats(psgsdf_ctx* c, int kind, psgsdf_step_stats* st);
int run_loop(psgsdf_ctx* c, int flags, LoopState& L, int max_iters, bool full, psgsdf_iter_stats* stats, int stats_cap, int* n_done, int* result,
             psgsdf_iter_cb on_iter, void* user);
int do_upsample(psgsdf_ctx* c);

}
```

### psgradientsdf_amd/csrc/loop.hip

```cpp
#include "engine_internal.h"
#include <climits>

namespace psge {

constexpr int kCgfSumsHost = 7;
void cgf_shape(int nblk, int* G, int* rows) {
    nblk = std::max(1, nblk);
    int r = 1, cap = kCgfMaxBlocks;
    if (const char* e = getenv("PSGSDF_PCG_ROWS")) { int v = atoi(e); if (v >= 1 && v <= 2) r = v; }
    if (const char* e = getenv("PSGSDF_PCG_BLOCKS")) { int v = atoi(e); if (v > 0 && v <= kCgfMaxBlocks) cap = v; }
    const int per = (nblk + r - 1) / r;
    const int trips = (per + cap - 1) / cap;
    *G = (per + trips - 1) / trips; *rows = r;
}

bool cgf_solve_shape(psgsdf_ctx* c, int* G, int* rows_per_wg, bool any_ranks) {
    if (!c->pcg_persist || c->persist_off || (c->n_ranks > 1 && !c->xr_ready && !any_ranks) || !c->band.col16 || !c->fuse_pcg_init || c->num_cu <= 0 || band_blocks(c) > kPcgMaxBlocks) return false;
    const int n = c->row1 - c->row0, cap = std::min(c->num_cu, kSolveMaxBlocksHost);
    if (n <= 0) return false;
    int g = std::min(cap, (n + kSolveThreadsHost - 1) / kSolveThreadsHost);
    g = std::max(8, g / 8 * 8);
    if (g > cap) g = cap;
    const int per = ((n + g - 1) / g + 63) / 64 * 64;
    const int r = (per + kSolveThreadsHost - 1) / kSolveThreadsHost;
    if (r > kSolveMaxRowsHost || cgf_solve_max_blocks(r) < 1) return false;
    *G = g; *rows_per_wg = per;
    return true;
}

int pcg_solve(psgsdf_ctx* c, SweepArgs& a, int* iters_out, int* success_out, double* err_out,
              const std::function<void(const double*)>& tail, bool gate_on_converged, bool* tail_ran) {
    const int S = c->band.S;
    if (tail_ran) *tail_ran = false;
    if (a.row1 <= a.row0) { *iters_out = 0; *success_out = 1; *err_out = 0; c->last_cg_iters = 0; return 0; }
    int cap = c->set.cg_max_it > 0 ? c->set.cg_max_it : 2 * S;
    if (cap > c->pcg_cap) cap = c->pcg_cap;
    int G, rows;
    if (a.pcg_gran && cgf_solve_shape(c, &G, &rows)) {
        SweepArgs as = a;
        auto fold_now = [&] { fold_by_kernel(c, as.fold); };
        if (slab_mode(c) && !xs_active(c)) fold_now();
        if (c->mbox_used + (size_t)kSolveMbSlots > c->mbox_n) { fold_now(); int rc = flush(c); if (rc) return rc; }
        { int rc = mg_commit(c); if (rc) return rc; }
        const size_t off = c->mbox_used; c->mbox_used += kSolveMbSlots;
        volatile double* st = c->mbox + off;
        const unsigned long long key = (++c->mbox_serial << 8) | 0x80u;
        st[3] = NAN; st[4] = 0.0;
        const int inject = (c->fault_solve > 0 && ++c->solves_seen == c->fault_solve) ? -7 : 0;
        const XrArgs* xr = (c->n_ranks > 1 && c->xr_ready && as.pcg_asm) ? &c->xr_args : nullptr;
        if (xr) {
            c->xr_solves++;
            c->xr_args.epoch = (unsigned)(c->xr_solves & (long long)kXrEpochMask);
            if (c->xr_args.epoch == 0) {
                HIPCHK(c, hipMemsetAsync(c->xr, 0, sizeof(double) * kXrDoubles, c->stream));
                HIPCHK(c, hipMemsetAsync(c->mg_ext, 0, sizeof(double), c->stream));
                int rc = comm_allreduce(c, c->mg_ext, 1); if (rc) return rc;
            }
        }
        as.pcg_epoch = ++c->pcg_solve_serial;
        timed(c, "pcg_solve", [&] { launch_cgf_solve(as, c->pcg_sc, c->pcg_gran, G, rows, cap, c->mbox_dev + off, key, inject, c->stream, xr); });
        if (tail && !c->profiling) { tail(c->pcg_sc + (gate_on_converged ? 2 : 1)); if (tail_ran) *tail_ran = true; }
        const bool chk = c->mbox_check;
        auto landed = [st, key, chk] {
            const double s3 = st[3];
            if (std::isnan(s3)) return false;
            return !chk || (dbits(st[0]) ^ dbits(st[1]) ^ dbits(st[2]) ^ dbits(s3) ^ dbits(st[4])) == key;
        };
        const int w = wait_mapped(c, landed, "pcg_solve");
        if (w < 0) return w;
        if (!landed()) HIPCHK(c, hipStreamSynchronize(c->stream));
        if (!landed()) return fail(c, PSGSDF_ERR_DEVICE, "the PCG kernel published nothing");
        if (w == 0 && !c->pending_fold.n) { int rc = deliver(c); if (rc) return rc; }
        if (st[3] != 1.0) {
            HIPCHK(c, hipStreamSynchronize(c->stream));
            if (!c->persist_fallbacks++) fprintf(stderr, "psgsdf: the persistent distance solve gave up waiting (status %g, %d workgroups%s): %s  Continuing with the per-pass kernels.\n", (double)st[3], G, xr ? ", cross-rank" : "",
                                                 xr ? "a neighbour rank's hand-off did not arrive in time." : "is another process holding CUs of this device?");
            c->persist_off = true;
            a.pcg_asm = 0; a.pcg_apply = 0; a.pcg_gran = nullptr; a.pcg_gran_n = 0; a.fold.n = 0;
            timed(c, "assemble", [&] { launch_assemble(a, c->stream); });
            if (tail_ran) *tail_ran = false;
            return pcg_solve(c, a, iters_out, success_out, err_out, tail, gate_on_converged, tail_ran);
        }
        const float rhsN = (float)st[2];
        if (rhsN == 0.f) { *iters_out = 0; *success_out = 1; *err_out = 0; c->last_cg_iters = 0; return 0; }
        const double err = sqrt((double)(float)st[1] / (double)rhsN);
        *iters_out = (int)st[0]; *err_out = err; *success_out = err <= (double)FLT_EPSILON;
        c->last_cg_iters = *iters_out;
        return 0;
    }
    cgf_shape(band_blocks(c), &G, &rows);
    if (!a.pcg_fuse_init) timed(c, "pcg_init", [&] { launch_cgf_init(a, c->pcg_sc, c->pcg_part, G, c->stream); });
    const bool mr = slab_mode(c);
    SweepArgs ap = a;
    if (mr) {
        int rc = mg_commit(c); if (rc) return rc;
        launch_cgf_sum(c->pcg_part, a.pcg_fuse_init ? a.pcg_init_blocks : G, -1, c->mg_ext, c->stream);
        if ((rc = comm_allreduce(c, c->mg_ext, 1))) return rc;
        ap.ext = c->mg_ext;
    }
    int chunk = std::min(64, std::max(4, c->last_cg_iters + 2));
    int k = 0, iters = -1;
    float rhsN = 0, rn2_last = 0, threshold = 0;
    while (true) {
        const int n = std::min(chunk, cap + 1 - k);
        if (c->mbox_used + (size_t)n > c->mbox_n) { int rc = flush(c); if (rc) return rc; }
        const size_t off = c->mbox_used; c->mbox_used += n;
        volatile double* st = c->mbox + off;
        for (int q = 0; q < n; ++q) st[q] = -1.0;
        for (int q = 0; q < n; ++q) {
            if (mr) { int rc = comm_halo(c, c->band.rec[(k + q + 1) & 1], 1, 4); if (rc) return rc; }
// ... 477 lines not shown
```

### psgradientsdf_amd/csrc/pcg.hip

```cpp
#include "device_common.h"

namespace psg {

__device__ __forceinline__ float pcg_threshold(float rhsNorm2) { return fmaxf(FLT_EPSILON * FLT_EPSILON * rhsNorm2, FLT_MIN); }


template <int N> struct PartLoads { double ld[kCgfMaxBlocks / kBlock][N]; };
template <int N>
__device__ __forceinline__ void block_total_issue(double* const* src, int n, PartLoads<N>& pl) {
#pragma unroll
    for (int j = 0; j < kCgfMaxBlocks / kBlock; ++j) {
        const int i = threadIdx.x + j * kBlock;
#pragma unroll
        for (int q = 0; q < N; ++q) pl.ld[j][q] = i < n ? src[q][i] : 0.0;
    }
}
template <int N>
__device__ __forceinline__ void block_total_finish(const PartLoads<N>& pl, double* red , double* out) {
    double v[8];
#pragma unroll
    for (int q = 0; q < 8; ++q) v[q] = 0.0;
#pragma unroll
    for (int q = 0; q < N; ++q) {
        v[q] = pl.ld[0][q];
#pragma unroll
        for (int j = 1; j < kCgfMaxBlocks / kBlock; ++j) v[q] += pl.ld[j][q];
    }
    const int lane = threadIdx.x & 63, w = threadIdx.x >> 6;
    if constexpr (N > 2) {
        double t0, t1; wave_sum8(v, t0, t1);
        __syncthreads();
        wave_sum8_store<kBlock / 64>(t0, t1, red, w);
    } else {
#pragma unroll
        for (int q = 0; q < N; ++q) v[q] = wave_sum(v[q]);
        __syncthreads();
        if (lane == 0) {
#pragma unroll
            for (int q = 0; q < N; ++q) red[q * (kBlock / 64) + w] = v[q];
        }
    }
    __syncthreads();
#pragma unroll
    for (int q = 0; q < N; ++q) {
        double s = 0;
#pragma unroll
        for (int i = 0; i < kBlock / 64; ++i) s += red[q * (kBlock / 64) + i];
        out[q] = s;
    }
}
template <int N>
__device__ __forceinline__ void block_total_n(double* const* src, int n, double* red , double* out) {
    PartLoads<N> pl;
    block_total_issue<N>(src, n, pl);
    block_total_finish<N>(pl, red, out);
}
template <int N>
__device__ __forceinline__ void block_part_store_n(const double* vin, double* const* dst, double* red , int slot) {
    static_assert(N > 2 && N <= 8, "reduce-scatter of up to eight sums");
    double v[8];
#pragma unroll
    for (int q = 0; q < 8; ++q) v[q] = q < N ? vin[q] : 0.0;
    const int w = threadIdx.x >> 6;
    double t0, t1; wave_sum8(v, t0, t1);
    __syncthreads();
    wave_sum8_store<kBlock / 64>(t0, t1, red, w);
    __syncthreads();
    if (threadIdx.x < N) {
        double s = 0;
        for (int i = 0; i < (int)(blockDim.x >> 6); ++i) s += red[threadIdx.x * (kBlock / 64) + i];
        dst[threadIdx.x][slot] = s;
    }
}

__global__ void __launch_bounds__(kBlock) k_cgf_init(SweepArgs a, double* fs, double* part) {
    __shared__ double red[kBlock / 64];
    const Band& b = a.b;
    double bb = 0;
    for (int i = a.row0 + blockIdx.x * blockDim.x + threadIdx.x; i < a.row1; i += gridDim.x * blockDim.x) {
        float dg = b.H[i];
        if (a.damping != 0.0f) dg += a.damping * dg;
        const float inv = dg != 0.f ? 1.0f / dg : 1.0f;
        const float r = b.rhs[i];
// ... 509 lines not shown
            if (k > 0 && !rhs_zero) x[u] = x[u] + alpha_prev * me[u].z;
            if (stop) continue;
            const float r_i = me[u].x - alpha_prev * me[u].y;
            const float z_i = me[u].w * r_i;
            const float p_i = z_i + beta * me[u].z;
            const float tt = (float)(A1[u] - (double)alpha_prev * A2[u] + (double)beta * A3[u]);
            me[u] = make_float4(r_i, tt, p_i, me[u].w);
            if (live[u]) {
                if (xcd_local) rout[row[u]] = me[u]; else store16_sc1(rout + row[u], me[u]);
                push_record(k & 1, row[u] - a.row0, me[u]);
                const double rd = (double)r_i, td = (double)tt, iv = (double)me[u].w;
                s[0] += (double)p_i * td; s[1] += iv * rd * td; s[2] += iv * td * td; s[3] += rd * td; s[4] += td * td;
                s[5] += rd * (double)z_i; s[6] += rd * rd;
            }
        }
        if (stop) break;
        if (force_passes == -7 && k == 2 && lb == 1) { status = 2; break; }
        SOLVE_STAMP(4);
        double sv[8];
#pragma unroll
        for (int q = 0; q < 8; ++q) sv[q] = q < kCgfSums ? s[q] : ((ASM && k == 0) ? bb_thread : 0.0);
        double t0, t1; wave_sum8(sv, t0, t1);
        asm volatile("s_waitcnt vmcnt(0)" ::: "memory");
        wave_sum8_store<kSolveThreads / 64>(t0, t1, red, tid >> 6);
        __syncthreads();
        SOLVE_STAMP(5);
        if (tid < kCgfSums || (ASM && k == 0 && tid == 7)) {
            double tot = 0;
            for (int i = 0; i < kSolveThreads / 64; ++i) tot += red[tid * (kSolveThreads / 64) + i];
            double* gq = gran + (size_t)(k & 1) * kSolveGranPlanes * kSolveMaxBlocks + (size_t)tid * kSolveMaxBlocks + lb;
            __hip_atomic_store(gq, gran_tag(tot, (unsigned)(k + 1) & 3u), __ATOMIC_RELAXED, __HIP_MEMORY_SCOPE_AGENT);
        }
        if (MR && tid == 64) peer_tag(k & 1, xr_tag(1.0, etag0 | ((unsigned)(k + 1) & 3u)));
        __syncthreads();
        SOLVE_STAMP(6);
        if (force_passes > 0 && k == 8 && tid == 0) fs[16 + lb] = (double)wall_clock64();
    }
#undef SOLVE_STAMP
#pragma unroll
    for (int u = 0; u < R; ++u) if (live[u]) b.x[row[u]] = x[u];
    if (a.pcg_apply) {
        const bool z0 = rhsNorm2 == 0.f;
        const bool ok_all = status == 1 && (z0 || sqrt((double)rr_cur / (double)rhsNorm2) <= (double)FLT_EPSILON);
        const bool apply = status == 1 && (a.pcg_apply == 1 || ok_all);
        double cnt = 0;
        if (apply) {
#pragma unroll
            for (int u = 0; u < R; ++u) if (live[u] && (double)fabsf(x[u]) < sqrt(3.0) * (double)a.grid.vs) { b.dist[row[u]] -= x[u]; cnt += 1.0; }
        }
        cnt = wave_sum(cnt);
        __syncthreads();
        if ((tid & 63) == 0) red[tid >> 6] = cnt;
        __syncthreads();
        double* slot = PART(a, SC_ACCEPT);
        if (tid == 0) { double t = 0; for (int i = 0; i < kSolveThreads / 64; ++i) t += red[i]; slot[lb] = t; }
        for (int i = G + lb * kSolveThreads + tid; i < a.acc.PB; i += G * kSolveThreads) slot[i] = 0.0;
    }
    if (lb == 0 && tid == 0) {
        const bool rhs_zero = rhsNorm2 == 0.f;
        const bool ok = status == 1 && (rhs_zero || sqrt((double)rr_cur / (double)rhsNorm2) <= (double)FLT_EPSILON);
        int iters = 0;
        if (!rhs_zero && k > 0) iters = (rr_cur < thr) ? k - 1 : k;
        fs[1] = status == 1 ? (double)(k + 1) : 0.0; fs[2] = ok ? 1.0 : 0.0;
        const double m0 = (double)iters, m1 = (double)rr_cur, m2 = (double)rhsNorm2, m3 = (double)status;
        mb[0] = m0; mb[1] = m1; mb[2] = m2;
        __threadfence_system();
        mb[3] = m3;
        if (mb_key) reinterpret_cast<unsigned long long*>(mb)[4] = (unsigned long long)(__double_as_longlong(m0) ^ __double_as_longlong(m1) ^ __double_as_longlong(m2) ^ __double_as_longlong(m3)) ^ mb_key;
        __threadfence_system();
    }
}

constexpr int kCgpSums = 3;
constexpr int kCgpMaxRows = 4;
#ifndef PSG_CGP_DEPTH
#define PSG_CGP_DEPTH 2
#endif
constexpr int kCgpDepth = PSG_CGP_DEPTH;
__device__ __forceinline__ void store8_sc1(double* p, double v) { asm volatile("global_store_dwordx2 %0, %1, off sc1\n\ts_nop 1" :: "v"(p), "v"(v) : "memory"); }
__device__ __forceinline__ void store8_sys(double* p, double v) { asm volatile("global_store_dwordx2 %0, %1, off sc0 sc1\n\ts_nop 1" :: "v"(p), "v"(v) : "memory"); }

__device__ __forceinline__ double m_tag(double v, unsigned tag) { return __longlong_as_double((long long)(((unsigned long long)__double_as_longlong(v) & ~15ull) | tag)); }
__device__ __forceinline__ unsigned m_tag_of(double v) { return (unsigned)((unsigned long long)__double_as_longlong(v) & 15ull); }
template <int R, bool MR, bool TM = false>
__global__ void __launch_bounds__(kSolveThreads, 2) k_cgp_solve(SweepArgs a, double* fs, double* gran, int rows_per_wg, int kmax, double* mb, unsigned long long mb_key, int force_passes, XrArgs xr) {
    __shared__ double red[8 * kSolveThreads / 64];
    __shared__ int s_abort;
    constexpr bool kFast = TM;
    __shared__ double red2[kFast ? 2 * 8 * kSolveThreads / 64 : 1];
    __shared__ double red3[(kFast && MR) ? 8 * kSolveThreads / 64 : 1];
    __shared__ int s_ab3[3];
#define CGP_ABORT (*(kFast ? &s_ab3[(k + 3) % 3] : &s_abort))
    __shared__ int s_foreign;
    const Band& b = a.b;
    const int G = gridDim.x, tid = threadIdx.x;
    const int my_xcc = (int)__builtin_amdgcn_s_getreg((20 << 0) | (0 << 6) | (3 << 11));
    bool xcd_local = false;
    const int lb = (G % 8 == 0) ? (int)(blockIdx.x % 8) * (G / 8) + (int)(blockIdx.x / 8) : (int)blockIdx.x;
    const int plane = b.Spad * 4;
    const __amdgpu_buffer_rsrc_t rC = __builtin_amdgcn_make_buffer_rsrc((void*)b.colp, 0, (kNQ - 1) / 2 * plane, 0x00020000);
    double* const recd[2] = {(double*)b.rec[0], (double*)b.rec[1]};
    const int own_n = a.row1 - a.row0;
    const int wg_first = lb * rows_per_wg, wg_last = min(own_n, wg_first + rows_per_wg) - 1;
    const bool cut_lo = MR && xr.give_lo > 0 && wg_first < xr.give_lo && wg_first < own_n;
    const bool cut_hi = MR && xr.give_hi > 0 && wg_last >= own_n - xr.give_hi && wg_first < own_n;
    const int hi_first_wg = MR ? max(0, own_n - xr.give_hi) / rows_per_wg : 0;
    double* const xr_me = MR ? xr.region[xr.rank] : nullptr;
    const unsigned etag0 = MR ? (xr.epoch & kXrEpochMask) << 2 : 0u;
    constexpr int kLocalSpins = MR ? (1 << 24) : (1 << 22);
    auto peer_tag = [&](int buf, double v) {
        if (cut_lo && lb < kXrPeerTags) __hip_atomic_store(xr.region[xr.rank - 1] + kXrPtag + (1 * 3 + buf) * kXrPeerTags + lb, v, __ATOMIC_RELAXED, __HIP_MEMORY_SCOPE_SYSTEM);
        if (cut_hi && lb - hi_first_wg < kXrPeerTags) __hip_atomic_store(xr.region[xr.rank + 1] + kXrPtag + (0 * 3 + buf) * kXrPeerTags + (lb - hi_first_wg), v, __ATOMIC_RELAXED, __HIP_MEMORY_SCOPE_SYSTEM);
    };
    const int lo_row0 = MR && xr.lo_rec[0] ? (int)(xr.lo_rec[0] - xr.lo_base[0]) : 0;
    auto push_record = [&](int buf, int rel, double v) {
        if (MR && rel < xr.give_lo) store8_sys((double*)xr.lo_base[buf] + lo_row0 + rel, v);
        if (MR && rel >= own_n - xr.give_hi) store8_sys((double*)xr.hi_rec[buf] + (rel - (own_n - xr.give_hi)), v);
    };
    auto raise_abort = [&] {
        __hip_atomic_store(fs + 3, 1.0, __ATOMIC_RELAXED, __HIP_MEMORY_SCOPE_AGENT);
        if (MR) for (int r = 0; r < xr.n_ranks; ++r) __hip_atomic_store(xr.region[r] + kXrAbort, 1.0, __ATOMIC_RELAXED, __HIP_MEMORY_SCOPE_SYSTEM);
    };
    float* hs = (float*)psg_dyn_smem;
    const unsigned mepoch = TM ? (1u + a.pcg_epoch % 3u) << 2 : 0u;
    unsigned cp[R][(kNQ - 1) / 2]; int row[R]; bool live[R];
    double x[R], r[R], w[R], z[R], sv[R], pv[R]; float inv[R];
    if (a.fold.n != 0 && blockIdx.x == 0) {
        double ftot[4] = {0.0, 0.0, 0.0, 0.0};
        for (int sl = 0; sl < a.fold.n; ++sl) {
            const double* part = PART(a, a.fold.id[sl]);
            double v = 0;
            if (tid < kBlock) for (int i = tid; i < a.fold.nblk; i += kBlock) v += part[i];
            v = wave_sum(v);
            __syncthreads();
            if ((tid & 63) == 0) red[tid >> 6] = v;
            __syncthreads();
            if (tid == 0) { double t = 0; for (int i = 0; i < kBlock / 64; ++i) t += red[i]; ftot[sl] = t; }
        }
        if (tid < 64) {
            if (a.fold.xf) fold_exchange(a.fold.xf, a.fold.xf_epoch, a.fold.n, ftot);
            if (tid == 0) {
                for (int sl = 0; sl < a.fold.n; ++sl) mbox_put(a.fold.out, a.fold.n, sl, ftot[sl], a.fold.key);
                mbox_commit(a.fold.key);
            }
        }
        __syncthreads();
    }
#pragma unroll
    for (int u = 0; u < R; ++u) {
        const int i = a.row0 + lb * rows_per_wg + u * kSolveThreads + tid;
        live[u] = u * kSolveThreads + tid < rows_per_wg && i < a.row1; row[u] = live[u] ? i : a.row1 - 1;
        double acc[kNQ], rhs;
        assemble_row_regs(a, row[u], acc, rhs);
#pragma unroll
        for (int q = 0; q < kNQ; ++q) {
            float hv = (float)acc[q];
            if (q == 0 && a.damping != 0.0f) hv += a.damping * hv;
            hs[(u * kNQ + q) * kSolveThreads + tid] = hv;
        }
        float dg = (float)acc[0];
        if (a.damping != 0.0f) dg += a.damping * dg;
        inv[u] = dg != 0.f ? 1.0f / dg : 1.0f;
        r[u] = live[u] ? (double)(float)rhs : 0.0;
        x[u] = 0.0; z[u] = 0.0; sv[u] = 0.0; pv[u] = 0.0; w[u] = 0.0;
        if (live[u]) {
            const double u0 = (double)inv[u] * r[u];
            if (TM) { const double ut = m_tag(u0, mepoch | 0u); __hip_atomic_store(recd[1] + row[u], ut, __ATOMIC_RELAXED, __HIP_MEMORY_SCOPE_AGENT); push_record(1, row[u] - a.row0, ut); }
            else { store8_sc1(recd[1] + row[u], u0); push_record(1, row[u] - a.row0, u0); }
        }
#pragma unroll
        for (int wd = 0; wd < (kNQ - 1) / 2; ++wd) cp[u][wd] = (unsigned)__builtin_amdgcn_raw_buffer_load_b32(rC, row[u] * 4, wd * plane, 0);
    }
    asm volatile("s_waitcnt vmcnt(0)" ::: "memory");
    __syncthreads();
    if (tid == 0) { __hip_atomic_store(gran + (size_t)(kSolveGranPlanes + 7) * kSolveMaxBlocks + lb, (double)(1 + my_xcc), __ATOMIC_RELAXED, __HIP_MEMORY_SCOPE_AGENT); if (MR && !TM) peer_tag(2, xr_tag(1.0, etag0 | 1u)); }
    float rhsNorm2 = 0.f, thr = 0.f, rr_cur = 0.f;
    double gamma_old = 0.0, alpha = 0.0;
    int k = -1, status = 1;
    const int first = lb * rows_per_wg, last = first + rows_per_wg - 1;
    const int nlo = max(0, (first - b.reach) / rows_per_wg), nhi = min(G - 1, (last + b.reach) / rows_per_wg);
    const bool need_lo = MR && xr.need_lo > 0 && wg_first < b.reach, need_hi = MR && xr.need_hi > 0 && wg_last + b.reach >= own_n;
#define SOLVE_STAMP(j) do { if (force_passes > 0 && k == 8 && tid == 0 && (lb == 0 || lb == (G * 9) / 16)) mb[8 + (lb ? 8 : 0) + (j)] = (double)wall_clock64(); } while (0)
    for (;; ++k) {
        SOLVE_STAMP(0);
        const unsigned want = (unsigned)(k + 1) & 3u;
        const double* gp = gran + (size_t)(k & 1) * kSolveGranPlanes * kSolveMaxBlocks;
#pragma unroll
        for (int u = 0; u < R; ++u)
#pragma unroll
            for (int wd = 0; wd < (kNQ - 1) / 2; ++wd) asm volatile("" : "+v"(cp[u][wd]));
        if (!kFast || k < 0) {
            if (tid == 0) { s_abort = 0; s_ab3[0] = 0; s_ab3[1] = 0; s_ab3[2] = 0; if (k < 0) s_foreign = 0; }
            __syncthreads();
        }
        if (!TM && tid <= nhi - nlo && !((a.pcg_xcd_local >> 3) & 2)) {
            int spins = 0;
            const double* wp = k >= 0 ? gp + nlo + tid : gran + (size_t)(kSolveGranPlanes + 7) * kSolveMaxBlocks + nlo + tid;
            double seen = 0.0;
            while (k >= 0 ? gran_tag_of(seen = __hip_atomic_load(wp, __ATOMIC_RELAXED, __HIP_MEMORY_SCOPE_AGENT)) != want : (seen = __hip_atomic_load(wp, __ATOMIC_RELAXED, __HIP_MEMORY_SCOPE_AGENT)) == 0.0) {
                __builtin_amdgcn_s_sleep(1);
                if (++spins > kLocalSpins || __hip_atomic_load(fs + 3, __ATOMIC_RELAXED, __HIP_MEMORY_SCOPE_AGENT) != 0.0) { CGP_ABORT = 1; break; }
            }
            if (k < 0 && (int)seen != 1 + my_xcc) s_foreign = 1;
        }
        if (MR && !TM) {
            const int side = tid >= 128 ? 1 : 0, j = tid - (side ? 128 : 64);
            if (tid >= 64 && tid < 192 && j < (side ? xr.wait_hi : xr.wait_lo) && (side ? need_hi : need_lo)) {
                int spins = 0;
                const double* wp = xr_me + kXrPtag + (side * 3 + (k >= 0 ? (k & 1) : 2)) * kXrPeerTags + j;
                const unsigned wantx = etag0 | (k >= 0 ? want : 1u);
                while (xr_tag_of(__hip_atomic_load(wp, __ATOMIC_RELAXED, __HIP_MEMORY_SCOPE_SYSTEM)) != wantx) {
                    __builtin_amdgcn_s_sleep(1);
                    if (++spins > (1 << 24) || __hip_atomic_load(fs + 3, __ATOMIC_RELAXED, __HIP_MEMORY_SCOPE_AGENT) != 0.0 || __hip_atomic_load(xr_me + kXrAbort, __ATOMIC_RELAXED, __HIP_MEMORY_SCOPE_SYSTEM) != 0.0) { CGP_ABORT = 1; break; }
                }
            }
        }
        if (!TM) {
            __syncthreads();
            if (CGP_ABORT) { if (tid == 0) raise_abort(); status = 2; break; }
            if (tid == 0) { if (MR) __builtin_amdgcn_fence(__ATOMIC_ACQUIRE, ""); else __builtin_amdgcn_fence(__ATOMIC_ACQUIRE, "agent"); }
            if (k < 0) xcd_local = (a.pcg_xcd_local & 1) && !s_foreign;
            __syncthreads();
        }
        SOLVE_STAMP(1);
        if (force_passes > 0 && k == 9 && tid == 0) fs[16 + 1536 + lb] = (double)wall_clock64();
        const double* __restrict__ rin = recd[k >= 0 ? (k & 1) : 1];
        const int abl = (a.pcg_xcd_local >> 3) & 7;
        double nres[R];
        double ob[kCgpDepth][9];
        auto issue = [&](int t) {
            const int u = t >> 1, j0 = (t & 1) * 9;
#pragma unroll
            for (int j = 0; j < 9; ++j) {
                const int jj = j0 + j; const int pk = (int)cp[u][jj >> 1];
                constexpr unsigned kInPlane = (1u << 0) | (1u << 1) | (1u << 2) | (1u << 3) | (1u << 6) | (1u << 7) | (1u << 12) | (1u << 13);
                if ((abl & 4) && ((kInPlane >> jj) & 1u)) { ob[t % kCgpDepth][j] = 0.0; continue; }
                const int srow = row[u] + ((abl & 1) ? 0 : ((jj & 1) ? (pk >> 16) : ((pk << 16) >> 16)));
                const double* src = rin + srow;
                if (TM && MR && (srow < a.row0 || srow >= a.row1)) ob[t % kCgpDepth][j] = __hip_atomic_load(src, __ATOMIC_RELAXED, __HIP_MEMORY_SCOPE_SYSTEM);
                else ob[t % kCgpDepth][j] = TM ? __hip_atomic_load(src, __ATOMIC_RELAXED, __HIP_MEMORY_SCOPE_AGENT) : *src;
            }
        };
        double v[8];
#pragma unroll
        for (int q = 0; q < 8; ++q) v[q] = 0.0;
        auto prefetch_sums = [&] {
            if (k >= 0 && (a.pcg_xcd_local & 2) && tid < G) {
#pragma unroll
                for (int q = 0; q < kCgpSums; ++q) v[q] = __hip_atomic_load(gp + (size_t)q * kSolveMaxBlocks + tid, __ATOMIC_RELAXED, __HIP_MEMORY_SCOPE_AGENT);
            }
        };
#pragma unroll
        for (int t = 0; t < kCgpDepth && t < 2 * R; ++t) issue(t);
        if (2 * R - 1 - kCgpDepth < 0) { __builtin_amdgcn_sched_barrier(0); prefetch_sums(); __builtin_amdgcn_sched_barrier(0); }
        double acc = 0;
#pragma unroll
        for (int t = 0; t < 2 * R; ++t) {
            const int u = t >> 1, j0 = (t & 1) * 9;
            const float* hrow = hs + (size_t)u * kNQ * kSolveThreads + tid;
            if (!(t & 1)) { const double mine = (double)inv[u] * (k >= 0 ? w[u] : r[u]); acc = (double)hrow[0] * mine; }
            if (TM) {
                const unsigned wantm = mepoch | want;
#pragma unroll
                for (int j = 0; j < 9; ++j) {
                    if (m_tag_of(ob[t % kCgpDepth][j]) == wantm) continue;
                    const int jj = j0 + j; const int pk = (int)cp[u][jj >> 1];
                    if ((abl & 4) && ((0x30cfu >> jj) & 1u)) continue;
                    const double* src = rin + (row[u] + ((jj & 1) ? (pk >> 16) : ((pk << 16) >> 16)));
                    int spins = 0; double vv;
                    do {
                        __builtin_amdgcn_s_sleep(1);
                        vv = MR ? __hip_atomic_load(src, __ATOMIC_RELAXED, __HIP_MEMORY_SCOPE_SYSTEM) : __hip_atomic_load(src, __ATOMIC_RELAXED, __HIP_MEMORY_SCOPE_AGENT);
                        if (++spins > kLocalSpins || ((spins & 255) == 0 && (__hip_atomic_load(fs + 3, __ATOMIC_RELAXED, __HIP_MEMORY_SCOPE_AGENT) != 0.0 || (MR && __hip_atomic_load(xr_me + kXrAbort, __ATOMIC_RELAXED, __HIP_MEMORY_SCOPE_SYSTEM) != 0.0)))) { CGP_ABORT = 1; break; }
                    } while (m_tag_of(vv) != wantm);
                    ob[t % kCgpDepth][j] = vv;
                }
            }
#pragma unroll
            for (int j = 0; j < 9; ++j) acc += (double)hrow[(j0 + j + 1) * kSolveThreads] * ob[t % kCgpDepth][j];
            asm volatile("" : "+v"(acc));
            if (t & 1) nres[u] = acc;
            __builtin_amdgcn_sched_barrier(0);
            if (t + kCgpDepth < 2 * R) issue(t + kCgpDepth);
            if (t == 2 * R - 1 - kCgpDepth) prefetch_sums();
            __builtin_amdgcn_sched_barrier(0);
        }
        SOLVE_STAMP(2);
        if (force_passes > 0 && k == 9 && tid == 0) { fs[16 + 1024 + lb] = (double)wall_clock64(); fs[16 + 768 + lb] = (double)my_xcc; fs[16 + 1792 + lb] = (double)(gran_tag_of(v[0]) == want && gran_tag_of(v[1]) == want && gran_tag_of(v[2]) == want); }
        double beta = 0.0;
        bool stop = false;
        if (k >= 0) {
            auto poll3 = [&](const double* base, bool prefetched) {
                int spins = 0;
                bool ok = prefetched && gran_tag_of(v[0]) == want && gran_tag_of(v[1]) == want && gran_tag_of(v[2]) == want;
                while (!ok) {
                    if (spins) __builtin_amdgcn_s_sleep(1);
                    if (++spins > kLocalSpins || __hip_atomic_load(fs + 3, __ATOMIC_RELAXED, __HIP_MEMORY_SCOPE_AGENT) != 0.0) { CGP_ABORT = 1; break; }
                    ok = true;
#pragma unroll
                    for (int q = 0; q < kCgpSums; ++q) { v[q] = __hip_atomic_load(base + (size_t)q * kSolveMaxBlocks, __ATOMIC_RELAXED, __HIP_MEMORY_SCOPE_AGENT); ok = ok && gran_tag_of(v[q]) == want; }
                }
            };
            if (tid < G) poll3(gp + tid, (a.pcg_xcd_local & 2) != 0);
            { const double v4[4] = {v[0], v[1], v[2], 0.0}; wave_sum4_store<kSolveThreads / 64>(wave_sum4(v4), red, tid >> 6); }
            __syncthreads();
            if (CGP_ABORT) { if (tid == 0) raise_abort(); status = 2; break; }
            double t[kCgpSums];
#pragma unroll
            for (int q = 0; q < kCgpSums; ++q) { double s_ = 0; for (int i = 0; i < kSolveThreads / 64; ++i) s_ += red[q * (kSolveThreads / 64) + i]; t[q] = s_; }
            if (!kFast) __syncthreads();
            if (MR) {
                const int pb = k & 1;
                if (lb == 0 && tid < kCgpSums) {
                    const double mine = xr_tag(t[tid], etag0 | want);
                    for (int rk = 0; rk < xr.n_ranks; ++rk) __hip_atomic_store(xr.region[rk] + kXrRankGran + (pb * 8 + tid) * kXrMaxRanks + xr.rank, mine, __ATOMIC_RELAXED, __HIP_MEMORY_SCOPE_SYSTEM);
                }
                double rv[8];
#pragma unroll
                for (int q = 0; q < 8; ++q) rv[q] = 0.0;
                if (tid < xr.n_ranks) {
                    int spins = 0; bool ok = false;
                    while (!ok) {
                        ok = true;
#pragma unroll
                        for (int q = 0; q < kCgpSums; ++q) { rv[q] = __hip_atomic_load(xr_me + kXrRankGran + (pb * 8 + q) * kXrMaxRanks + tid, __ATOMIC_RELAXED, __HIP_MEMORY_SCOPE_SYSTEM); ok = ok && xr_tag_of(rv[q]) == (etag0 | want); }
                        if (!ok) {
                            __builtin_amdgcn_s_sleep(1);
                            if (++spins > (1 << 24) || __hip_atomic_load(fs + 3, __ATOMIC_RELAXED, __HIP_MEMORY_SCOPE_AGENT) != 0.0 || __hip_atomic_load(xr_me + kXrAbort, __ATOMIC_RELAXED, __HIP_MEMORY_SCOPE_SYSTEM) != 0.0) { CGP_ABORT = 1; break; }
                        }
                    }
                }
                double* const redR = kFast ? red3 : red;
                double r0, r1; wave_sum8(rv, r0, r1);
                wave_sum8_store<kSolveThreads / 64>(r0, r1, redR, tid >> 6);
                __syncthreads();
                if (CGP_ABORT) { if (tid == 0) raise_abort(); status = 2; break; }
#pragma unroll
                for (int q = 0; q < kCgpSums; ++q) t[q] = redR[q * (kSolveThreads / 64)];
                if (!kFast) __syncthreads();
            }
            if (k == 0) { rhsNorm2 = (float)t[2]; thr = pcg_threshold(rhsNorm2); if (lb == 0 && tid == 0) fs[0] = t[2]; }
            rr_cur = (float)t[2];
            const bool rhs_zero = rhsNorm2 == 0.f;
            stop = force_passes > 0 ? k >= force_passes : (rhs_zero || k == kmax || (k > 0 && rr_cur < thr));
            if (!stop) {
                beta = k > 0 ? t[0] / gamma_old : 0.0;
                alpha = t[0] / (k > 0 ? t[1] - beta * t[0] / alpha : t[1]);
                gamma_old = t[0];
            }
        }
        SOLVE_STAMP(3);
        if (force_passes > 0 && k == 9 && tid == 0) fs[16 + 256 + lb] = fs[16 + 512 + lb] = (double)wall_clock64();
        if (stop) break;
        if (force_passes == -7 && k == 2 && lb == 1) { status = 2; break; }
        double s[8];
#pragma unroll
        for (int q = 0; q < 8; ++q) s[q] = 0.0;
#pragma unroll
        for (int u = 0; u < R; ++u) {
            double ui = (double)inv[u] * r[u];
            if (k < 0) w[u] = nres[u];
            else {
                z[u] = nres[u] + beta * z[u];
                sv[u] = w[u] + beta * sv[u];
                pv[u] = ui + beta * pv[u];
                x[u] = x[u] + alpha * pv[u];
                r[u] = r[u] - alpha * sv[u];
                w[u] = w[u] - alpha * z[u];
                ui = (double)inv[u] * r[u];
            }
            const double mnext = (double)inv[u] * w[u];
            if (live[u]) {
                s[0] += r[u] * ui; s[1] += w[u] * ui; s[2] += r[u] * r[u];
                double* dst = recd[(k + 1) & 1] + row[u];
                if (TM) { const double mt = m_tag(mnext, mepoch | ((unsigned)(k + 2) & 3u)); __hip_atomic_store(dst, mt, __ATOMIC_RELAXED, __HIP_MEMORY_SCOPE_AGENT); push_record((k + 1) & 1, row[u] - a.row0, mt); }
                else {
                    if (!xcd_local) store8_sc1(dst, mnext);
                    *dst = mnext;
                    push_record((k + 1) & 1, row[u] - a.row0, mnext);
                }
            }
        }
        SOLVE_STAMP(4);
        const double s4[4] = {s[0], s[1], s[2], 0.0};
        const double tE = wave_sum4(s4);
        if (!TM) asm volatile("s_waitcnt vmcnt(0)" ::: "memory");
        double* const redE = kFast ? red2 + ((k + 1) & 1) * (8 * kSolveThreads / 64) : red;
        wave_sum4_store<kSolveThreads / 64>(tE, redE, tid >> 6);
        __syncthreads();
        if (TM && CGP_ABORT) { if (tid == 0) raise_abort(); status = 2; break; }
        if (kFast && tid == 0) s_ab3[(k + 5) % 3] = 0;
        SOLVE_STAMP(5);
        if (tid < kCgpSums) {
            double tot = 0;
            for (int i = 0; i < kSolveThreads / 64; ++i) tot += redE[tid * (kSolveThreads / 64) + i];
            double* gq = gran + (size_t)((k + 1) & 1) * kSolveGranPlanes * kSolveMaxBlocks + (size_t)tid * kSolveMaxBlocks + lb;
            __hip_atomic_store(gq, gran_tag(tot, (unsigned)(k + 2) & 3u), __ATOMIC_RELAXED, __HIP_MEMORY_SCOPE_AGENT);
        }
        if (MR && !TM && tid == 64) peer_tag((k + 1) & 1, xr_tag(1.0, etag0 | ((unsigned)(k + 2) & 3u)));
        if (!kFast) __syncthreads();
        SOLVE_STAMP(6);
        if (force_passes > 0 && k == 8 && tid == 0) fs[16 + lb] = (double)wall_clock64();
        if (force_passes > 0 && k == 9 && tid == 0) fs[16 + 1280 + lb] = (double)wall_clock64();
    }
#undef SOLVE_STAMP
#undef CGP_ABORT
    float xf[R];
#pragma unroll
    for (int u = 0; u < R; ++u) { xf[u] = (float)x[u]; if (live[u]) b.x[row[u]] = xf[u]; }
    if (a.pcg_apply) {
        const bool z0 = rhsNorm2 == 0.f;
        const bool ok_all = status == 1 && (z0 || sqrt((double)rr_cur / (double)rhsNorm2) <= (double)FLT_EPSILON);
        const bool apply = status == 1 && (a.pcg_apply == 1 || ok_all);
        double cnt = 0;
        if (apply) {
#pragma unroll
            for (int u = 0; u < R; ++u) if (live[u] && (double)fabsf(xf[u]) < sqrt(3.0) * (double)a.grid.vs) { b.dist[row[u]] -= xf[u]; cnt += 1.0; }
        }
        cnt = wave_sum(cnt);
        __syncthreads();
        if ((tid & 63) == 0) red[tid >> 6] = cnt;
        __syncthreads();
        double* slot = PART(a, SC_ACCEPT);
        if (tid == 0) { double t = 0; for (int i = 0; i < kSolveThreads / 64; ++i) t += red[i]; slot[lb] = t; }
        for (int i = G + lb * kSolveThreads + tid; i < a.acc.PB; i += G * kSolveThreads) slot[i] = 0.0;
    }
    if (lb == 0 && tid == 0) {
        const bool rhs_zero = rhsNorm2 == 0.f;
        const bool ok = status == 1 && (rhs_zero || sqrt((double)rr_cur / (double)rhsNorm2) <= (double)FLT_EPSILON);
        int iters = 0;
        if (!rhs_zero && k > 0) iters = (rr_cur < thr) ? k - 1 : k;
        fs[1] = status == 1 ? (double)(k + 1) : 0.0; fs[2] = ok ? 1.0 : 0.0;
        const double m0 = (double)iters, m1 = (double)rr_cur, m2 = (double)rhsNorm2, m3 = (double)status;
        mb[0] = m0; mb[1] = m1; mb[2] = m2;
        __threadfence_system();
        mb[3] = m3;
        if (mb_key) reinterpret_cast<unsigned long long*>(mb)[4] = (unsigned long long)(__double_as_longlong(m0) ^ __double_as_longlong(m1) ^ __double_as_longlong(m2) ^ __double_as_longlong(m3)) ^ mb_key;
        __threadfence_system();
    }
}
static size_t cgf_solve_lds(int rows) { return sizeof(float) * (size_t)rows * kNQ * kSolveThreads; }
static size_t cgp_solve_lds(int rows) { return cgf_solve_lds(rows); }
template <int R, bool ASM, bool MR> static int cgf_solve_prepare() {
    static int per_cu = -1;
    if (per_cu >= 0) return per_cu;
    per_cu = 0;
    if (hipFuncSetAttribute((const void*)k_cgf_solve<R, ASM, MR>, hipFuncAttributeMaxDynamicSharedMemorySize, (int)cgf_solve_lds(R)) != hipSuccess) return per_cu;
    int n = 0;
    if (hipOccupancyMaxActiveBlocksPerMultiprocessor(&n, k_cgf_solve<R, ASM, MR>, kSolveThreads, cgf_solve_lds(R)) == hipSuccess) per_cu = n;
    return per_cu;
}
template <int R, bool MR, bool TM = false> static int cgp_solve_prepare() {
    static int per_cu = -1;
    if (per_cu >= 0) return per_cu;
    per_cu = 0;
    if (hipFuncSetAttribute((const void*)k_cgp_solve<R, MR, TM>, hipFuncAttributeMaxDynamicSharedMemorySize, (int)cgp_solve_lds(R)) != hipSuccess) return per_cu;
    int n = 0;
    if (hipOccupancyMaxActiveBlocksPerMultiprocessor(&n, k_cgp_solve<R, MR, TM>, kSolveThreads, cgp_solve_lds(R)) == hipSuccess) per_cu = n;
    return per_cu;
}
template <int R> static int cgf_solve_prepare_both() {
    const int classic = std::min(std::min(cgf_solve_prepare<R, false, false>(), cgf_solve_prepare<R, true, false>()), cgf_solve_prepare<R, true, true>());
    if (R > kCgpMaxRows) return classic;
    return std::min(classic, std::min(std::min(cgp_solve_prepare<R, false>(), cgp_solve_prepare<R, false, true>()), std::min(cgp_solve_prepare<R, true>(), cgp_solve_prepare<R, true, true>())));
}
int cgf_solve_max_blocks(int rows) {
    return rows == 1 ? cgf_solve_prepare_both<1>() : rows == 2 ? cgf_solve_prepare_both<2>() : rows == 3 ? cgf_solve_prepare_both<3>() : cgf_solve_prepare_both<4>();
}
template <int R>
static void launch_cgf_solve_r(const SweepArgs& a, double* fs, double* gran, int G, int rows_per_wg, int kmax, double* mb, unsigned long long mb_key, int force_passes, hipStream_t s, const XrArgs* xr) {
    XrArgs none{};
    if (a.pcg_asm && a.pcg_pipe && R <= kCgpMaxRows) {
        if (xr && xr->n_ranks > 1 && a.pcg_pipe == 3) hipLaunchKernelGGL((k_cgp_solve<R, true, true>), dim3(G), dim3(kSolveThreads), cgp_solve_lds(R), s, a, fs, gran, rows_per_wg, kmax, mb, mb_key, force_passes, *xr);
        else if (xr && xr->n_ranks > 1) hipLaunchKernelGGL((k_cgp_solve<R, true>), dim3(G), dim3(kSolveThreads), cgp_solve_lds(R), s, a, fs, gran, rows_per_wg, kmax, mb, mb_key, force_passes, *xr);
        else if (a.pcg_pipe >= 2) { hipLaunchKernelGGL((k_cgp_solve<R, false, true>), dim3(G), dim3(kSolveThreads), cgp_solve_lds(R), s, a, fs, gran, rows_per_wg, kmax, mb, mb_key, force_passes, none); }
        else hipLaunchKernelGGL((k_cgp_solve<R, false>), dim3(G), dim3(kSolveThreads), cgp_solve_lds(R), s, a, fs, gran, rows_per_wg, kmax, mb, mb_key, force_passes, none);
        return;
    }
    if (xr && xr->n_ranks > 1 && a.pcg_asm) hipLaunchKernelGGL((k_cgf_solve<R, true, true>), dim3(G), dim3(kSolveThreads), cgf_solve_lds(R), s, a, fs, gran, rows_per_wg, kmax, mb, mb_key, force_passes, *xr);
    else if (a.pcg_asm) hipLaunchKernelGGL((k_cgf_solve<R, true, false>), dim3(G), dim3(kSolveThreads), cgf_solve_lds(R), s, a, fs, gran, rows_per_wg, kmax, mb, mb_key, force_passes, none);
    else hipLaunchKernelGGL((k_cgf_solve<R, false, false>), dim3(G), dim3(kSolveThreads), cgf_solve_lds(R), s, a, fs, gran, rows_per_wg, kmax, mb, mb_key, force_passes, none);
}
void launch_cgf_solve(const SweepArgs& a, double* fs, double* gran, int G, int rows_per_wg, int kmax, double* mb, unsigned long long mb_key, int force_passes, hipStream_t s, const XrArgs* xr) {
    const int rows = (rows_per_wg + kSolveThreads - 1) / kSolveThreads;
    if (rows == 1) launch_cgf_solve_r<1>(a, fs, gran, G, rows_per_wg, kmax, mb, mb_key, force_passes, s, xr);
    else if (rows == 2) launch_cgf_solve_r<2>(a, fs, gran, G, rows_per_wg, kmax, mb, mb_key, force_passes, s, xr);
    else if (rows == 3) launch_cgf_solve_r<3>(a, fs, gran, G, rows_per_wg, kmax, mb, mb_key, force_passes, s, xr);
    else launch_cgf_solve_r<4>(a, fs, gran, G, rows_per_wg, kmax, mb, mb_key, force_passes, s, xr);
}

__global__ void __launch_bounds__(kBlock) k_cgf_sum(double* part, int G, int k, double* __restrict__ out) {
    __shared__ double red[8 * kBlock / 64];
    if (k < 0) {
        double* src[1] = {fpart(part, -1, 6)}; double bb;
        block_total_n<1>(src, G, red, &bb);
        if (threadIdx.x == 0) out[0] = bb;
    } else {
        double* src[kCgfSums]; double t[kCgfSums];
#pragma unroll
        for (int q = 0; q < kCgfSums; ++q) src[q] = fpart(part, k, q);
        block_total_n<kCgfSums>(src, G, red, t);
        if (threadIdx.x < kCgfSums) out[threadIdx.x] = t[threadIdx.x];
    }
}
void launch_cgf_sum(double* part, int G, int k, double* out, hipStream_t s) {
    hipLaunchKernelGGL(k_cgf_sum, dim3(1), dim3(kBlock), 0, s, part, G, k, out);
}

__global__ void __launch_bounds__(kBlock) k_matvec(SweepArgs a, const float* x, float* y) {
    const Band& b = a.b;
    int i = blockIdx.x * blockDim.x + threadIdx.x;
    if (i >= b.S) return;
    double acc = 0;
    for (int q = 0; q < kNQ; ++q) {
        int c = q == 0 ? i : b.col[(size_t)q * b.Spad + i];
        if (c < 0) continue;
        acc += (double)b.H[(size_t)q * b.Spad + i] * (double)x[c];
    }
    y[i] = (float)acc;
}
void launch_matvec(const SweepArgs& a, const float* x, float* y, hipStream_t s) {
    if (a.row1 > a.row0) hipLaunchKernelGGL(k_matvec, dim3((a.row1 - a.row0 + kBlock - 1) / kBlock), dim3(kBlock), 0, s, a, x, y);
}
__global__ void __launch_bounds__(kBlock) k_apply_dist(SweepArgs a) {
    __shared__ double red[kBlock / 64];
    if (a.gate && *a.gate == 0.0) return;
    const Band& b = a.b;
    int j = a.row0 + blockIdx.x * blockDim.x + threadIdx.x;
    double cnt = 0;
    if (j < a.row1) {
        float d = b.x[j];
        if ((double)fabsf(d) < sqrt(3.0) * (double)a.grid.vs) { b.dist[j] -= d; cnt = 1.0; }
    }
    block_part_store(cnt, PART(a, SC_ACCEPT), red);
}
void launch_apply_dist(const SweepArgs& a, hipStream_t s) {
    if (a.row1 > a.row0) hipLaunchKernelGGL(k_apply_dist, dim3((a.row1 - a.row0 + kBlock - 1) / kBlock), dim3(kBlock), 0, s, a);
}

}
```

Before: 2910.

## Stage per-workgroup PCG neighbour window in LDS for persistent solve

```diff
diff --git a/__graft_entry__.py b/__graft_entry__.py
--- a/__graft_entry__.py
+++ b/__graft_entry__.py
@@ -23,7 +23,7 @@
     h = hashlib.sha256()
     for f in sorted(glob.glob(os.path.join(csrc, "*.hip")) + glob.glob(os.path.join(csrc, "*.h")) + glob.glob(os.path.join(ROOT, "psgradientsdf_amd", "host", "*.[ch]pp"))
                     + [os.path.join(csrc, "Makefile"), os.path.join(ROOT, "include", "psgsdf.h"), os.path.join(ROOT, "include", "psgsdf_render.h"),
-                       os.path.join(ROOT, "include", "psgsdf_mesh.h"), os.path.join(ROOT, "include", "psgsdf_fit.h")]):
+                       os.path.join(ROOT, "include", "psgsdf_mesh.h"), os.path.join(ROOT, "include", "psgsdf_fit.h"), os.path.join(ROOT, "include", "psgsdf_debug.h")]):
         h.update(os.path.relpath(f, ROOT).encode()); h.update(open(f, "rb").read())
     stamp = os.path.join(csrc, ".build_hash")
     clean = os.environ.get("PSGSDF_BUILD_CLEAN") == "1" or not os.path.exists(stamp) or open(stamp).read() != h.hexdigest() \
@@ -40,7 +40,7 @@
 
     for path in (capi.ENGINE_LIB, capi.ENGINE_LIB_DEV):
         lib = ctypes.CDLL(path)
-        missing = [s for s in _declared_symbols() + _declared_symbols("psgsdf_render.h") + _declared_symbols("psgsdf_mesh.h") + _declared_symbols("psgsdf_fit.h") if not hasattr(lib, s)]
+        missing = [s for s in _declared_symbols() + _declared_symbols("psgsdf_render.h") + _declared_symbols("psgsdf_mesh.h") + _declared_symbols("psgsdf_fit.h") + _declared_symbols("psgsdf_debug.h") if not hasattr(lib, s)]
         if missing:
             raise RuntimeError(f"{os.path.basename(path)} lacks {missing}")
 
diff --git a/include/psgsdf_debug.h b/include/psgsdf_debug.h
--- /dev/null
+++ b/include/psgsdf_debug.h
@@ -0,0 +1,13 @@
+#ifndef PSGSDF_DEBUG_H_
+#define PSGSDF_DEBUG_H_
+#include "psgsdf.h"
+#ifdef __cplusplus
+extern "C" {
+#endif
+
+int psgsdf_debug_solve_window(psgsdf_ctx* ctx, int32_t info[4], int32_t* table, int32_t* cols);
+
+#ifdef __cplusplus
+}
+#endif
+#endif
diff --git a/psgradientsdf_amd/capi.py b/psgradientsdf_amd/capi.py
--- a/psgradientsdf_amd/capi.py
+++ b/psgradientsdf_amd/capi.py
@@ -546,6 +546,16 @@
         self._check(self._fn("debug_time_pcg_solve")(self.ctx, C.c_int(passes), C.c_int(reps), C.byref(ms), shape, st), "debug_time_pcg_solve")
         return ms.value, (shape[0], shape[1]), [x for x in st]
 
+    def debug_solve_window(self, tables=True):
+        info = (C.c_int32 * 4)()
+        self._check(self._fn("debug_solve_window")(self.ctx, info, None, None), "debug_solve_window")
+        out = dict(G=info[0], rows_per_wg=info[1], S=info[2], active=bool(info[3]))
+        if tables:
+            tab = np.empty((info[0], 8), np.int32); cols = np.empty((18, info[2]), np.int32)
+            self._check(self._fn("debug_solve_window")(self.ctx, info, tab.ctypes.data_as(C.c_void_p), cols.ctypes.data_as(C.c_void_p)), "debug_solve_window")
+            out.update(table=tab, cols=cols)
+        return out
+
     def debug_sync_stats(self):
         out = (C.c_int64 * 8)()
         self._check(self._fn("debug_sync_stats")(self.ctx, out), "debug_sync_stats")
diff --git a/psgradientsdf_amd/csrc/api.hip b/psgradientsdf_amd/csrc/api.hip
--- a/psgradientsdf_amd/csrc/api.hip
+++ b/psgradientsdf_amd/csrc/api.hip
@@ -27,11 +27,11 @@
 
 static const char* const kKnobs[] = {
     "PSGSDF_PCG_POLL", "PSGSDF_SPECULATE", "PSGSDF_FOLD_IN_NEXT", "PSGSDF_FUSE_ALBEDO", "PSGSDF_FUSE_PCG_INIT", "PSGSDF_PCG_PERSIST", "PSGSDF_PCG_XCD_LOCAL",
-    "PSGSDF_PCG_FUSE_ASM", "PSGSDF_PCG_FUSE_APPLY", "PSGSDF_PCG_PIPELINE", "PSGSDF_PCG_TAGM", "PSGSDF_PCG_PREFETCH", "PSGSDF_PCG_COL16", "PSGSDF_PCG_ROWS", "PSGSDF_PCG_BLOCKS",
+    "PSGSDF_PCG_FUSE_ASM", "PSGSDF_PCG_FUSE_APPLY", "PSGSDF_PCG_PIPELINE", "PSGSDF_PCG_TAGM", "PSGSDF_PCG_PREFETCH", "PSGSDF_PCG_WINDOW", "PSGSDF_PCG_COL16", "PSGSDF_PCG_ROWS", "PSGSDF_PCG_BLOCKS",
     "PSGSDF_FM_SOLVE", "PSGSDF_FRAME_SOLVE", "PSGSDF_FM_ROWS", "PSGSDF_IMG_COMPACT", "PSGSDF_XCD_MAP", "PSGSDF_XCD_STRIPE",
     "PSGSDF_XR", "PSGSDF_XF", "PSGSDF_XS", "PSGSDF_XH", "PSGSDF_XR_MEM", "PSGSDF_XWAIT_LOG2", "PSGSDF_SPECULATE_MR", "PSGSDF_CU_MASK",
     "PSGSDF_WAIT_TIMEOUT_S", "PSGSDF_DESTROY_TIMEOUT_S", "PSGSDF_SOLVE_DUMP"};
-static const char* const kDevKnobs[] = {"PSGSDF_PCG_ABLATE", "PSGSDF_FAULT_SOLVE", "PSGSDF_FAULT_HALO", "PSGSDF_MBOX_CHECK"};
+static const char* const kDevKnobs[] = {"PSGSDF_PCG_ABLATE", "PSGSDF_FAULT_SOLVE", "PSGSDF_FAULT_HALO", "PSGSDF_MBOX_CHECK", "PSGSDF_PCG_WINDOW_CAP", "PSGSDF_PCG_SOLVE_WGS"};
 const char* psgsdf_last_error(const psgsdf_ctx* c) { return c ? c->err : "null context"; }
 
 int psgsdf_create(const psgsdf_grid_desc* grid, const float K[9], const psgsdf_settings* settings, int device, psgsdf_ctx** out) {
@@ -54,6 +54,7 @@
     if (const char* e = getenv("PSGSDF_PCG_PIPELINE")) c->pcg_pipeline = atoi(e) != 0;
     if (const char* e = getenv("PSGSDF_PCG_TAGM")) { c->pcg_tagm = atoi(e) != 0; c->pcg_tagm_mr = atoi(e) >= 2; }
     if (const char* e = getenv("PSGSDF_PCG_PREFETCH")) c->pcg_prefetch = atoi(e) != 0;
+    if (const char* e = getenv("PSGSDF_PCG_WINDOW")) c->pcg_window = atoi(e) != 0;
     if (const char* e = getenv("PSGSDF_FM_SOLVE")) { c->fm_solve = atoi(e) != 0; c->fm_solve_led = atoi(e) == 1; }
     if (const char* e = getenv("PSGSDF_FRAME_SOLVE")) c->frame_solve = (!strcmp(e, "eigen") || !strcmp(e, "1")) ? 1 : 0;
     if (const char* e = getenv("PSGSDF_XF")) c->xf_enable = atoi(e) != 0;
@@ -69,6 +70,8 @@
     if (const char* e = getenv("PSGSDF_MBOX_CHECK")) c->mbox_check = atoi(e) != 0;
     if (const char* e = getenv("PSGSDF_FAULT_SOLVE")) c->fault_solve = atoi(e);
     if (const char* e = getenv("PSGSDF_FAULT_HALO")) c->fault_halo = atoll(e);
+    if (const char* e = getenv("PSGSDF_PCG_WINDOW_CAP")) c->pcg_win_cap = atoll(e);
+    if (const char* e = getenv("PSGSDF_PCG_SOLVE_WGS")) c->pcg_solve_wgs = atoi(e);
 #endif
     for (const char* k : kKnobs) if (const char* e = getenv(k)) c->tuning_env.emplace_back(k, e);
     for (const char* k : kDevKnobs) if (const char* e = getenv(k)) {
@@ -126,7 +129,7 @@
     free_dense(c);
     hipFree(c->vis_seq); hipFree(c->frame_idx); hipFree(c->img); hipFree(c->img8); hipFree(c->frames); hipFree(c->frames_undo); hipFree(c->led_light); hipFree(c->fs_stats);
     hipFree(c->band_mem); if (!c->leak_exported) hipFree(c->rec_mem); hipFree(c->obs_mem); hipFree(c->stage);
-    hipFree(c->ncache); hipFree(c->ntmp); hipFree(c->nout); hipFree(c->ndepth); hipFree(c->track_part); if (c->track_host) hipHostFree(c->track_host); hipFree(c->acc_frame); hipFree(c->frame_part); hipFree(c->frame_done); hipFree(c->part); hipFree(c->pcg_sc); hipFree(c->pcg_part); hipFree(c->pcg_gran); hipFree(c->d_total);
+    hipFree(c->ncache); hipFree(c->ntmp); hipFree(c->nout); hipFree(c->ndepth); hipFree(c->track_part); if (c->track_host) hipHostFree(c->track_host); hipFree(c->acc_frame); hipFree(c->frame_part); hipFree(c->frame_done); hipFree(c->part); hipFree(c->pcg_sc); hipFree(c->pcg_part); hipFree(c->pcg_gran); hipFree(c->pcg_win); hipFree(c->d_total);
     for (void* p : c->xo_host) if (p) hipHostFree(p);
     if (c->pin_stage) hipHostFree(c->pin_stage);
     if (c->host_buf) hipHostFree(c->host_buf);
diff --git a/psgradientsdf_amd/csrc/api_debug.hip b/psgradientsdf_amd/csrc/api_debug.hip
--- a/psgradientsdf_amd/csrc/api_debug.hip
+++ b/psgradientsdf_amd/csrc/api_debug.hip
@@ -1,4 +1,5 @@
 #include "engine_internal.h"
+#include "../../include/psgsdf_debug.h"
 
 using namespace psge;
 
@@ -241,6 +242,27 @@
     return PSGSDF_OK;
 }
 
+int psgsdf_debug_solve_window(psgsdf_ctx* c, int32_t info[4], int32_t* table, int32_t* cols) {
+    if (!c || !c->inited || !info) return fail(c, PSGSDF_ERR_STATE, "init first");
+    HIPCHK(c, hipSetDevice(c->device));
+    int G = 0, rows = 0;
+    if (!cgf_solve_shape(c, &G, &rows)) return fail(c, PSGSDF_ERR_UNSUPPORTED, "the persistent solve does not apply to this context");
+    const int S = c->band.S, Sp = c->band.Spad;
+    info[0] = G; info[1] = rows; info[2] = S; info[3] = (c->pcg_win_on && !c->persist_off && c->pcg_win_G == G && c->pcg_win_rows == rows) ? 1 : 0;
+    if (table) {
+        if (!c->pcg_win || c->pcg_win_bytes == 0) return fail(c, PSGSDF_ERR_UNSUPPORTED, "no segment table was built for this band");
+        HIPCHK(c, hipMemcpyAsync(table, c->pcg_win, sizeof(int32_t) * 8 * G, hipMemcpyDeviceToHost, c->stream));
+    }
+    if (cols) {
+        std::vector<unsigned> pk((size_t)9 * Sp);
+        HIPCHK(c, hipMemcpyAsync(pk.data(), c->band.colp, sizeof(unsigned) * pk.size(), hipMemcpyDeviceToHost, c->stream));
+        HIPCHK(c, hipStreamSynchronize(c->stream));
+        for (int jj = 0; jj < 18; ++jj) for (int i = 0; i < S; ++i) { const int w = (int)pk[(size_t)(jj >> 1) * Sp + i]; cols[(size_t)jj * S + i] = i + ((jj & 1) ? (w >> 16) : ((w << 16) >> 16)); }
+    }
+    HIPCHK(c, hipStreamSynchronize(c->stream));
+    return PSGSDF_OK;
+}
+
 int psgsdf_debug_sync_stats(psgsdf_ctx* c, int64_t out[8]) {
     if (!c || !out) return PSGSDF_ERR_ARG;
     out[0] = c->mbox_checked; out[1] = c->mbox_late; out[2] = c->persist_fallbacks + (c->img_compacted ? 1000000LL : 0); out[3] = c->spec_windows * 1000000LL + c->spec_undos;
@@ -261,11 +283,11 @@
     char buf[1024];
     snprintf(buf, sizeof(buf), "\"pcg_poll\": %d, \"speculate\": %d, \"speculate_mr\": %d, \"fold_in_next\": %d, \"fuse_albedo\": %d, \"fuse_pcg_init\": %d, \"pcg_persist\": %d, \"pcg_pipeline\": %d, \"pcg_tagm\": %d, "
              "\"pcg_prefetch\": %d, \"pcg_fuse_asm\": %d, \"pcg_fuse_apply\": %d, \"pcg_xcd_local\": %d, \"fm_solve\": %d, \"fm_solve_led\": %d, \"frame_solve\": \"%s\", \"img_compact\": %d, \"xcd_map\": %d, "
-             "\"xr\": %d, \"xf\": %d, \"xs\": %d, \"xh\": %d, \"xr_mem_kind\": %d, \"xwait_log2\": %d, \"cu_mask\": [%d, %d], \"mbox_check\": %d, \"pcg_ablate\": %d, \"fault_solve\": %d, \"fault_halo\": %lld",
+             "\"xr\": %d, \"xf\": %d, \"xs\": %d, \"xh\": %d, \"xr_mem_kind\": %d, \"xwait_log2\": %d, \"cu_mask\": [%d, %d], \"mbox_check\": %d, \"pcg_ablate\": %d, \"fault_solve\": %d, \"fault_halo\": %lld, \"pcg_window\": %d, \"pcg_window_bytes\": %d",
              (int)c->pcg_poll, (int)c->speculate, (int)c->speculate_mr, (int)c->fold_in_next, (int)c->fuse_albedo, (int)c->fuse_pcg_init, (int)c->pcg_persist, (int)c->pcg_pipeline, (c->pcg_pipeline && c->pcg_tagm) ? (c->n_ranks > 1 ? (c->pcg_tagm_mr ? 2 : 0) : 1) : 0,
              (int)c->pcg_prefetch, (int)c->pcg_fuse_asm, (int)c->pcg_fuse_apply, (int)c->pcg_xcd_local, (int)c->fm_solve, (int)c->fm_solve_led, c->frame_solve == 1 ? "eigen" : "ldlt", (int)c->img_compact, c->xcd_map,
              (int)c->xr_enable, (int)c->xf_enable, (int)c->xs_enable, (int)c->xh_enable, c->xr_mem_kind, (int)lround(log2((double)c->xwait_spins)), c->cu_mask_lo, c->cu_mask_hi,
-             (int)c->mbox_check, c->pcg_ablate, c->fault_solve, c->fault_halo);
+             (int)c->mbox_check, c->pcg_ablate, c->fault_solve, c->fault_halo, (c->pcg_win_on && !c->persist_off) ? 1 : 0, c->pcg_win_bytes);
     o += buf; o += "}";
     if (c->n_ranks > 1) {
         snprintf(buf, sizeof(buf), ", \"xr_probe\": {\"rank\": %d, \"n_ranks\": %d, \"kind_chosen\": %d, \"stale_mappings\": %lld, \"fine_grained\": {\"tried\": %lld, \"stale_records_from_lower\": %lld, \"expired_waits_lower\": %lld, \"expired_waits_upper\": %lld}, "
diff --git a/psgradientsdf_amd/csrc/engine.h b/psgradientsdf_amd/csrc/engine.h
--- a/psgradientsdf_amd/csrc/engine.h
+++ b/psgradientsdf_amd/csrc/engine.h
@@ -128,6 +128,8 @@
     FrameP* fm_frames; float* fm_undo; double* fm_e_out; unsigned long long fm_e_key;
     const double* gate;
     const double* ext;
+    const int* pcg_win;
+    int pcg_win_bytes, pcg_win_G, pcg_win_rows;
 };
 
 constexpr int kXrMaxRanks = 32;
@@ -200,6 +202,9 @@
 constexpr int kSolveGranPlanes = 8;
 constexpr int kSolveThreadsHost = 512, kSolveMaxBlocksHost = 256, kSolveMaxRowsHost = 4, kSolveMbSlots = 24;
 int cgf_solve_max_blocks(int rows);
+void launch_solve_window_table(const Band& b, int row0, int row1, int G, int rows_per_wg, int* tab, hipStream_t s);
+int cgp_window_batch();
+bool cgp_window_fits(int rows_per_wg, size_t win_bytes, size_t* cap);
 void launch_cgf_solve(const SweepArgs& a, double* fs, double* gran, int G, int rows_per_wg, int kmax, double* mb, unsigned long long mb_key, int force_passes, hipStream_t s, const XrArgs* xr = nullptr);
 void launch_areg_tables(const DenseView& d, const GridP& g, const SweepArgs& a, hipStream_t s);
 void launch_areg_build(const SweepArgs& a, hipStream_t s);
diff --git a/psgradientsdf_amd/csrc/engine.hip b/psgradientsdf_amd/csrc/engine.hip
--- a/psgradientsdf_amd/csrc/engine.hip
+++ b/psgradientsdf_amd/csrc/engine.hip
@@ -41,6 +41,7 @@
     a.xcd_map = c->xcd_map; a.xf = nullptr; a.xf_epoch = 0; a.fm_led_light = nullptr; a.vm_order = c->vm_order;
     a.fm_solve = 0; a.fm_frames = nullptr; a.fm_undo = nullptr; a.fm_e_out = nullptr; a.fm_e_key = 0;
     a.pcg_part = c->pcg_part; a.pcg_fs = c->pcg_sc; a.pcg_fuse_init = 0; a.pcg_init_blocks = 0; a.pcg_gran = nullptr; a.pcg_gran_n = 0; a.pcg_asm = 0; a.pcg_epoch = 0; a.pcg_pipe = c->pcg_pipeline ? (c->pcg_tagm ? (c->n_ranks <= 1 ? 2 : (c->pcg_tagm_mr ? 3 : 1)) : 1) : 0; a.pcg_apply = 0; a.pcg_xcd_local = (c->pcg_xcd_local ? 1 : 0) | (c->pcg_prefetch ? 2 : 0) | (c->pcg_ablate << 3);
+    a.pcg_win = c->pcg_win_on ? c->pcg_win : nullptr; a.pcg_win_bytes = c->pcg_win_bytes; a.pcg_win_G = c->pcg_win_G; a.pcg_win_rows = c->pcg_win_rows;
     a.ar = c->ar; a.ar.weight = c->reg_r;
     a.model = c->set.model; a.quirks = c->set.ref_quirks;
     a.reg_n = c->reg_n; a.reg_l = c->reg_l;
@@ -400,6 +401,7 @@
         }
         c->mbox_used = 0; c->deferred.clear(); c->mg_segs.clear();
     }
+    { int rc = solve_window_prepare(c); if (rc) return rc; }
     return ensure_host_buf(c, (size_t)SC_COUNT * c->PB + (size_t)c->F * kFrameRow + 4096 + 64);
 }
 
diff --git a/psgradientsdf_amd/csrc/engine_internal.h b/psgradientsdf_amd/csrc/engine_internal.h
--- a/psgradientsdf_amd/csrc/engine_internal.h
+++ b/psgradientsdf_amd/csrc/engine_internal.h
@@ -81,6 +81,11 @@
     bool pcg_tagm = true;
     int pcg_ablate = 0;
     bool pcg_prefetch = true;
+    bool pcg_window = true;
+    int* pcg_win = nullptr;
+    bool pcg_win_on = false; int pcg_win_bytes = 0, pcg_win_G = 0, pcg_win_rows = 0;
+    long long pcg_win_cap = -1;
+    int pcg_solve_wgs = 0;
     bool pcg_pipeline = true;
     bool pcg_fuse_apply = true;
     bool pcg_xcd_local = true;
@@ -278,6 +283,7 @@
 
 struct LoopState { float E, E_n, E_l, E_prev; int laplacian_reg; float E_r; };
 void cgf_shape(int nblk, int* G, int* rows);
+int solve_window_prepare(psgsdf_ctx* c);
 bool cgf_solve_shape(psgsdf_ctx* c, int* G, int* rows, bool any_ranks = false);
 int pcg_solve(psgsdf_ctx* c, SweepArgs& a, int* iters_out, int* success_out, double* err_out,
               const std::function<void(const double*)>& tail = nullptr, bool gate_on_converged = true, bool* tail_ran = nullptr);
diff --git a/psgradientsdf_amd/csrc/loop.hip b/psgradientsdf_amd/csrc/loop.hip
--- a/psgradientsdf_amd/csrc/loop.hip
+++ b/psgradientsdf_amd/csrc/loop.hip
@@ -16,8 +16,10 @@
 
 bool cgf_solve_shape(psgsdf_ctx* c, int* G, int* rows_per_wg, bool any_ranks) {
     if (!c->pcg_persist || c->persist_off || (c->n_ranks > 1 && !c->xr_ready && !any_ranks) || !c->band.col16 || !c->fuse_pcg_init || c->num_cu <= 0 || band_blocks(c) > kPcgMaxBlocks) return false;
-    const int n = c->row1 - c->row0, cap = std::min(c->num_cu, kSolveMaxBlocksHost);
+    const int n = c->row1 - c->row0;
+    int cap = std::min(c->num_cu, kSolveMaxBlocksHost);
     if (n <= 0) return false;
+    if (c->pcg_solve_wgs >= 8 && c->pcg_solve_wgs < cap) cap = c->pcg_solve_wgs;
     int g = std::min(cap, (n + kSolveThreadsHost - 1) / kSolveThreadsHost);
     g = std::max(8, g / 8 * 8);
     if (g > cap) g = cap;
@@ -26,6 +28,37 @@
     if (r > kSolveMaxRowsHost || cgf_solve_max_blocks(r) < 1) return false;
     *G = g; *rows_per_wg = per;
     return true;
+}
+
+int solve_window_prepare(psgsdf_ctx* c) {
+    c->pcg_win_on = false; c->pcg_win_bytes = 0; c->pcg_win_G = 0; c->pcg_win_rows = 0;
+    int G = 0, rows = 0;
+    if (!c->pcg_window || c->n_ranks > 1 || c->pcg_ablate || !c->pcg_pipeline || !c->pcg_tagm || !c->pcg_fuse_asm || !cgf_solve_shape(c, &G, &rows)) return PSGSDF_OK;
+    if ((rows + kSolveThreadsHost - 1) / kSolveThreadsHost > 3) return PSGSDF_OK;
+    constexpr int kSlots = 8;
+    if (!c->pcg_win) HIPCHK(c, hipMalloc(&c->pcg_win, sizeof(int) * kSlots * kSolveMaxBlocksHost));
+    launch_solve_window_table(c->band, c->row0, c->row1, G, rows, c->pcg_win, c->stream);
+    std::vector<int> tab((size_t)kSlots * G);
+    HIPCHK(c, hipMemcpyAsync(tab.data(), c->pcg_win, sizeof(int) * tab.size(), hipMemcpyDeviceToHost, c->stream));
+    HIPCHK(c, hipStreamSynchronize(c->stream));
+    long long max_rows = 0, max_halo = 0;
+    for (int g = 0; g < G; ++g) {
+        const int* t = tab.data() + (size_t)kSlots * g;
+        long long n = 0;
+        for (int k = 0; k < 3; ++k) {
+            if (t[2 * k + 1] >= t[2 * k] && (t[2 * k] < 0 || t[2 * k + 1] >= c->band.S)) return fail(c, PSGSDF_ERR_DEVICE, "solve window: segment [%d, %d] of workgroup %d outside the band", t[2 * k], t[2 * k + 1], g);
+            n += std::max(0, t[2 * k + 1] - t[2 * k] + 1);
+        }
+        const int first = c->row0 + g * rows, last = std::min(c->row1, first + rows) - 1;
+        max_rows = std::max(max_rows, n); max_halo = std::max(max_halo, n - std::max(0, last - first + 1));
+    }
+    const size_t bytes = sizeof(double) * (size_t)max_rows;
+    size_t cap = 0;
+    c->pcg_win_bytes = (int)bytes;
+    if (c->pcg_win_cap >= 0 && (long long)bytes > c->pcg_win_cap) return PSGSDF_OK;
+    if (max_halo > cgp_window_batch() || !cgp_window_fits(rows, bytes, &cap)) return PSGSDF_OK;
+    c->pcg_win_on = true; c->pcg_win_G = G; c->pcg_win_rows = rows;
+    return PSGSDF_OK;
 }
 
 int pcg_solve(psgsdf_ctx* c, SweepArgs& a, int* iters_out, int* success_out, double* err_out,
diff --git a/psgradientsdf_amd/csrc/pcg.hip b/psgradientsdf_amd/csrc/pcg.hip
--- a/psgradientsdf_amd/csrc/pcg.hip
+++ b/psgradientsdf_amd/csrc/pcg.hip
@@ -1,4 +1,5 @@
 #include "device_common.h"
+#include <climits>
 
 namespace psg {
 
@@ -674,7 +675,10 @@
 
 __device__ __forceinline__ double m_tag(double v, unsigned tag) { return __longlong_as_double((long long)(((unsigned long long)__double_as_longlong(v) & ~15ull) | tag)); }
 __device__ __forceinline__ unsigned m_tag_of(double v) { return (unsigned)((unsigned long long)__double_as_longlong(v) & 15ull); }
-template <int R, bool MR, bool TM = false>
+constexpr int kWinBatch = 12;
+constexpr int kWinSlots = 8;
+__host__ __device__ inline int win_class(int jj) { int o[3]; q_offset(jj + 1, o); return o[2] == 0 ? 0 : (o[2] < 0 ? 1 : 2); }
+template <int R, bool MR, bool TM = false, bool WIN = false>
 __global__ void __launch_bounds__(kSolveThreads, 2) k_cgp_solve(SweepArgs a, double* fs, double* gran, int rows_per_wg, int kmax, double* mb, unsigned long long mb_key, int force_passes, XrArgs xr) {
     __shared__ double red[8 * kSolveThreads / 64];
     __shared__ int s_abort;
@@ -714,6 +718,21 @@
         if (MR) for (int r = 0; r < xr.n_ranks; ++r) __hip_atomic_store(xr.region[r] + kXrAbort, 1.0, __ATOMIC_RELAXED, __HIP_MEMORY_SCOPE_SYSTEM);
     };
     float* hs = (float*)psg_dyn_smem;
+    double* const win = reinterpret_cast<double*>(hs + (size_t)R * kNQ * kSolveThreads);
+    int woff[3] = {0, 0, 0}, w_own_at = 0, w_own_n = 0, w_halo = 0;
+    int hsrc[WIN ? kWinBatch : 1];
+    if constexpr (WIN) {
+        const int* tb = a.pcg_win + lb * kWinSlots;
+        const int lo0 = tb[0], n0 = max(0, tb[1] - tb[0] + 1), lo1 = tb[2], n1 = max(0, tb[3] - tb[2] + 1), lo2 = tb[4], n2 = max(0, tb[5] - tb[4] + 1);
+        woff[0] = -lo0; woff[1] = n0 - lo1; woff[2] = n0 + n1 - lo2;
+        w_own_n = max(0, wg_last - wg_first + 1); w_own_at = w_own_n > 0 ? a.row0 + wg_first - lo0 : 0;
+        w_halo = n0 + n1 + n2 - w_own_n;
+#pragma unroll
+        for (int i = 0; i < kWinBatch; ++i) {
+            const int e = i * kSolveThreads + tid, slot = e + (e >= w_own_at ? w_own_n : 0);
+            hsrc[i] = e < w_halo ? (slot < n0 ? slot + lo0 : (slot < n0 + n1 ? slot - n0 + lo1 : slot - n0 - n1 + lo2)) : -1;
+        }
+    }
     const unsigned mepoch = TM ? (1u + a.pcg_epoch % 3u) << 2 : 0u;
     unsigned cp[R][(kNQ - 1) / 2]; int row[R]; bool live[R];
     double x[R], r[R], w[R], z[R], sv[R], pv[R]; float inv[R];
@@ -765,6 +784,10 @@
     }
     asm volatile("s_waitcnt vmcnt(0)" ::: "memory");
     __syncthreads();
+    if constexpr (WIN) {
+#pragma unroll
+        for (int u = 0; u < R; ++u) if (live[u]) win[row[u] + woff[0]] = m_tag((double)inv[u] * r[u], mepoch | 0u);
+    }
     if (tid == 0) { __hip_atomic_store(gran + (size_t)(kSolveGranPlanes + 7) * kSolveMaxBlocks + lb, (double)(1 + my_xcc), __ATOMIC_RELAXED, __HIP_MEMORY_SCOPE_AGENT); if (MR && !TM) peer_tag(2, xr_tag(1.0, etag0 | 1u)); }
     float rhsNorm2 = 0.f, thr = 0.f, rr_cur = 0.f;
     double gamma_old = 0.0, alpha = 0.0;
@@ -819,20 +842,6 @@
         const double* __restrict__ rin = recd[k >= 0 ? (k & 1) : 1];
         const int abl = (a.pcg_xcd_local >> 3) & 7;
         double nres[R];
-        double ob[kCgpDepth][9];
-        auto issue = [&](int t) {
-            const int u = t >> 1, j0 = (t & 1) * 9;
-#pragma unroll
-            for (int j = 0; j < 9; ++j) {
-                const int jj = j0 + j; const int pk = (int)cp[u][jj >> 1];
-                constexpr unsigned kInPlane = (1u << 0) | (1u << 1) | (1u << 2) | (1u << 3) | (1u << 6) | (1u << 7) | (1u << 12) | (1u << 13);
-                if ((abl & 4) && ((kInPlane >> jj) & 1u)) { ob[t % kCgpDepth][j] = 0.0; continue; }
-                const int srow = row[u] + ((abl & 1) ? 0 : ((jj & 1) ? (pk >> 16) : ((pk << 16) >> 16)));
-                const double* src = rin + srow;
-                if (TM && MR && (srow < a.row0 || srow >= a.row1)) ob[t % kCgpDepth][j] = __hip_atomic_load(src, __ATOMIC_RELAXED, __HIP_MEMORY_SCOPE_SYSTEM);
-                else ob[t % kCgpDepth][j] = TM ? __hip_atomic_load(src, __ATOMIC_RELAXED, __HIP_MEMORY_SCOPE_AGENT) : *src;
-            }
-        };
         double v[8];
 #pragma unroll
         for (int q = 0; q < 8; ++q) v[q] = 0.0;
@@ -842,43 +851,111 @@
                 for (int q = 0; q < kCgpSums; ++q) v[q] = __hip_atomic_load(gp + (size_t)q * kSolveMaxBlocks + tid, __ATOMIC_RELAXED, __HIP_MEMORY_SCOPE_AGENT);
             }
         };
-#pragma unroll
-        for (int t = 0; t < kCgpDepth && t < 2 * R; ++t) issue(t);
-        if (2 * R - 1 - kCgpDepth < 0) { __builtin_amdgcn_sched_barrier(0); prefetch_sums(); __builtin_amdgcn_sched_barrier(0); }
-        double acc = 0;
-#pragma unroll
-        for (int t = 0; t < 2 * R; ++t) {
-            const int u = t >> 1, j0 = (t & 1) * 9;
-            const float* hrow = hs + (size_t)u * kNQ * kSolveThreads + tid;
-            if (!(t & 1)) { const double mine = (double)inv[u] * (k >= 0 ? w[u] : r[u]); acc = (double)hrow[0] * mine; }
-            if (TM) {
-                const unsigned wantm = mepoch | want;
+        if constexpr (!WIN) {
+            double ob[kCgpDepth][9];
+            auto issue = [&](int t) {
+                const int u = t >> 1, j0 = (t & 1) * 9;
 #pragma unroll
                 for (int j = 0; j < 9; ++j) {
-                    if (m_tag_of(ob[t % kCgpDepth][j]) == wantm) continue;
                     const int jj = j0 + j; const int pk = (int)cp[u][jj >> 1];
-                    if ((abl & 4) && ((0x30cfu >> jj) & 1u)) continue;
-                    const double* src = rin + (row[u] + ((jj & 1) ? (pk >> 16) : ((pk << 16) >> 16)));
-                    int spins = 0; double vv;
+                    constexpr unsigned kInPlane = (1u << 0) | (1u << 1) | (1u << 2) | (1u << 3) | (1u << 6) | (1u << 7) | (1u << 12) | (1u << 13);
+                    if ((abl & 4) && ((kInPlane >> jj) & 1u)) { ob[t % kCgpDepth][j] = 0.0; continue; }
+                    const int srow = row[u] + ((abl & 1) ? 0 : ((jj & 1) ? (pk >> 16) : ((pk << 16) >> 16)));
+                    const double* src = rin + srow;
+                    if (TM && MR && (srow < a.row0 || srow >= a.row1)) ob[t % kCgpDepth][j] = __hip_atomic_load(src, __ATOMIC_RELAXED, __HIP_MEMORY_SCOPE_SYSTEM);
+                    else ob[t % kCgpDepth][j] = TM ? __hip_atomic_load(src, __ATOMIC_RELAXED, __HIP_MEMORY_SCOPE_AGENT) : *src;
+                }
+            };
+#pragma unroll
+            for (int t = 0; t < kCgpDepth && t < 2 * R; ++t) issue(t);
+            if (2 * R - 1 - kCgpDepth < 0) { __builtin_amdgcn_sched_barrier(0); prefetch_sums(); __builtin_amdgcn_sched_barrier(0); }
+            double acc = 0;
+#pragma unroll
+            for (int t = 0; t < 2 * R; ++t) {
+                const int u = t >> 1, j0 = (t & 1) * 9;
+                const float* hrow = hs + (size_t)u * kNQ * kSolveThreads + tid;
+                if (!(t & 1)) { const double mine = (double)inv[u] * (k >= 0 ? w[u] : r[u]); acc = (double)hrow[0] * mine; }
+                if (TM) {
+                    const unsigned wantm = mepoch | want;
+#pragma unroll
+                    for (int j = 0; j < 9; ++j) {
+                        if (m_tag_of(ob[t % kCgpDepth][j]) == wantm) continue;
+                        const int jj = j0 + j; const int pk = (int)cp[u][jj >> 1];
+                        if ((abl & 4) && ((0x30cfu >> jj) & 1u)) continue;
+                        const double* src = rin + (row[u] + ((jj & 1) ? (pk >> 16) : ((pk << 16) >> 16)));
+                        int spins = 0; double vv;
+                        do {
+                            __builtin_amdgcn_s_sleep(1);
+                            vv = MR ? __hip_atomic_load(src, __ATOMIC_RELAXED, __HIP_MEMORY_SCOPE_SYSTEM) : __hip_atomic_load(src, __ATOMIC_RELAXED, __HIP_MEMORY_SCOPE_AGENT);
+                            if (++spins > kLocalSpins || ((spins & 255) == 0 && (__hip_atomic_load(fs + 3, __ATOMIC_RELAXED, __HIP_MEMORY_SCOPE_AGENT) != 0.0 || (MR && __hip_atomic_load(xr_me + kXrAbort, __ATOMIC_RELAXED, __HIP_MEMORY_SCOPE_SYSTEM) != 0.0)))) { CGP_ABORT = 1; break; }
+                        } while (m_tag_of(vv) != wantm);
+                        ob[t % kCgpDepth][j] = vv;
+                    }
+                }
+#pragma unroll
+                for (int j = 0; j < 9; ++j) acc += (double)hrow[(j0 + j + 1) * kSolveThreads] * ob[t % kCgpDepth][j];
+                asm volatile("" : "+v"(acc));
+                if (t & 1) nres[u] = acc;
+                __builtin_amdgcn_sched_barrier(0);
+                if (t + kCgpDepth < 2 * R) issue(t + kCgpDepth);
+                if (t == 2 * R - 1 - kCgpDepth) prefetch_sums();
+                __builtin_amdgcn_sched_barrier(0);
+            }
+        } else {
+            const unsigned wantm = mepoch | want;
+            double hv[kWinBatch];
+#pragma unroll
+            for (int i = 0; i < kWinBatch; ++i) {
+                hv[i] = 0.0;
+                if (i * kSolveThreads < w_halo && hsrc[i] >= 0) hv[i] = __hip_atomic_load(rin + hsrc[i], __ATOMIC_RELAXED, __HIP_MEMORY_SCOPE_AGENT);
+            }
+            __builtin_amdgcn_sched_barrier(0); prefetch_sums(); __builtin_amdgcn_sched_barrier(0);
+            bool gave_up = false;
+#pragma unroll
+            for (int i = 0; i < kWinBatch; ++i) {
+                if (i * kSolveThreads >= w_halo || hsrc[i] < 0) continue;
+                double vv = hv[i];
+                if (m_tag_of(vv) != wantm && !gave_up) {
+                    const double* src = rin + hsrc[i];
+                    int spins = 0;
                     do {
                         __builtin_amdgcn_s_sleep(1);
-                        vv = MR ? __hip_atomic_load(src, __ATOMIC_RELAXED, __HIP_MEMORY_SCOPE_SYSTEM) : __hip_atomic_load(src, __ATOMIC_RELAXED, __HIP_MEMORY_SCOPE_AGENT);
-                        if (++spins > kLocalSpins || ((spins & 255) == 0 && (__hip_atomic_load(fs + 3, __ATOMIC_RELAXED, __HIP_MEMORY_SCOPE_AGENT) != 0.0 || (MR && __hip_atomic_load(xr_me + kXrAbort, __ATOMIC_RELAXED, __HIP_MEMORY_SCOPE_SYSTEM) != 0.0)))) { CGP_ABORT = 1; break; }
+                        vv = __hip_atomic_load(src, __ATOMIC_RELAXED, __HIP_MEMORY_SCOPE_AGENT);
+                        if (++spins > kLocalSpins || ((spins & 255) == 0 && __hip_atomic_load(fs + 3, __ATOMIC_RELAXED, __HIP_MEMORY_SCOPE_AGENT) != 0.0)) { CGP_ABORT = 1; gave_up = true; break; }
                     } while (m_tag_of(vv) != wantm);
-                    ob[t % kCgpDepth][j] = vv;
-                }
-            }
-#pragma unroll
-            for (int j = 0; j < 9; ++j) acc += (double)hrow[(j0 + j + 1) * kSolveThreads] * ob[t % kCgpDepth][j];
-            asm volatile("" : "+v"(acc));
-            if (t & 1) nres[u] = acc;
-            __builtin_amdgcn_sched_barrier(0);
-            if (t + kCgpDepth < 2 * R) issue(t + kCgpDepth);
-            if (t == 2 * R - 1 - kCgpDepth) prefetch_sums();
-            __builtin_amdgcn_sched_barrier(0);
-        }
-        SOLVE_STAMP(2);
-        if (force_passes > 0 && k == 9 && tid == 0) { fs[16 + 1024 + lb] = (double)wall_clock64(); fs[16 + 768 + lb] = (double)my_xcc; fs[16 + 1792 + lb] = (double)(gran_tag_of(v[0]) == want && gran_tag_of(v[1]) == want && gran_tag_of(v[2]) == want); }
+                }
+                const int e = i * kSolveThreads + tid;
+                win[e + (e >= w_own_at ? w_own_n : 0)] = vv;
+            }
+        }
+        const bool pf_valid = gran_tag_of(v[0]) == want && gran_tag_of(v[1]) == want && gran_tag_of(v[2]) == want;
+        auto stamp_b = [&] {
+            SOLVE_STAMP(2);
+            if (force_passes > 0 && k == 9 && tid == 0) { fs[16 + 1024 + lb] = (double)wall_clock64(); fs[16 + 768 + lb] = (double)my_xcc; fs[16 + 1792 + lb] = (double)pf_valid; }
+        };
+        auto win_product = [&] {
+#pragma unroll
+            for (int u = 0; u < R; ++u) {
+                nres[u] = 0.0;
+                if (!live[u]) continue;
+                const float* hrow = hs + (size_t)u * kNQ * kSolveThreads + tid;
+                const double mine = (double)inv[u] * (k >= 0 ? w[u] : r[u]);
+                double acc = (double)hrow[0] * mine;
+#pragma unroll
+                for (int jj = 0; jj < kNQ - 1; ++jj) {
+                    const int pk = (int)cp[u][jj >> 1], d = (jj & 1) ? (pk >> 16) : ((pk << 16) >> 16), cls = win_class(jj);
+                    const int at = row[u] + ((cls != 0 && d == 0) ? woff[0] : d + woff[cls]);
+                    acc += (double)hrow[(jj + 1) * kSolveThreads] * win[at];
+                }
+                nres[u] = acc;
+            }
+        };
+        if constexpr (!WIN) stamp_b();
+        else if (k < 0) {
+            __syncthreads();
+            if (CGP_ABORT) { if (tid == 0) raise_abort(); status = 2; break; }
+            win_product(); stamp_b();
+        }
         double beta = 0.0;
         bool stop = false;
         if (k >= 0) {
@@ -897,6 +974,7 @@
             { const double v4[4] = {v[0], v[1], v[2], 0.0}; wave_sum4_store<kSolveThreads / 64>(wave_sum4(v4), red, tid >> 6); }
             __syncthreads();
             if (CGP_ABORT) { if (tid == 0) raise_abort(); status = 2; break; }
+            if constexpr (WIN) { win_product(); stamp_b(); }
             double t[kCgpSums];
 #pragma unroll
             for (int q = 0; q < kCgpSums; ++q) { double s_ = 0; for (int i = 0; i < kSolveThreads / 64; ++i) s_ += red[q * (kSolveThreads / 64) + i]; t[q] = s_; }
@@ -948,6 +1026,7 @@
         double s[8];
 #pragma unroll
         for (int q = 0; q < 8; ++q) s[q] = 0.0;
+        double mown[WIN ? R : 1];
 #pragma unroll
         for (int u = 0; u < R; ++u) {
             double ui = (double)inv[u] * r[u];
@@ -965,7 +1044,7 @@
             if (live[u]) {
                 s[0] += r[u] * ui; s[1] += w[u] * ui; s[2] += r[u] * r[u];
                 double* dst = recd[(k + 1) & 1] + row[u];
-                if (TM) { const double mt = m_tag(mnext, mepoch | ((unsigned)(k + 2) & 3u)); __hip_atomic_store(dst, mt, __ATOMIC_RELAXED, __HIP_MEMORY_SCOPE_AGENT); push_record((k + 1) & 1, row[u] - a.row0, mt); }
+                if (TM) { const double mt = m_tag(mnext, mepoch | ((unsigned)(k + 2) & 3u)); __hip_atomic_store(dst, mt, __ATOMIC_RELAXED, __HIP_MEMORY_SCOPE_AGENT); push_record((k + 1) & 1, row[u] - a.row0, mt); if constexpr (WIN) mown[u] = mt; }
                 else {
                     if (!xcd_local) store8_sc1(dst, mnext);
                     *dst = mnext;
@@ -981,6 +1060,10 @@
         wave_sum4_store<kSolveThreads / 64>(tE, redE, tid >> 6);
         __syncthreads();
         if (TM && CGP_ABORT) { if (tid == 0) raise_abort(); status = 2; break; }
+        if constexpr (WIN) {
+#pragma unroll
+            for (int u = 0; u < R; ++u) if (live[u]) win[row[u] + woff[0]] = mown[u];
+        }
         if (kFast && tid == 0) s_ab3[(k + 5) % 3] = 0;
         SOLVE_STAMP(5);
         if (tid < kCgpSums) {
@@ -1051,6 +1134,49 @@
     if (hipOccupancyMaxActiveBlocksPerMultiprocessor(&n, k_cgp_solve<R, MR, TM>, kSolveThreads, cgp_solve_lds(R)) == hipSuccess) per_cu = n;
     return per_cu;
 }
+__global__ void __launch_bounds__(kSolveThreads) k_solve_window_table(Band b, int row0, int row1, int rows_per_wg, int* __restrict__ tab) {
+    __shared__ int lo[3], hi[3];
+    const int lb = blockIdx.x, tid = threadIdx.x;
+    const int first = row0 + lb * rows_per_wg, last = min(row1, first + rows_per_wg) - 1;
+    if (tid < 3) { lo[tid] = (tid == 0 && first <= last) ? first : INT_MAX; hi[tid] = (tid == 0 && first <= last) ? last : -1; }
+    __syncthreads();
+    int l[3] = {INT_MAX, INT_MAX, INT_MAX}, h[3] = {-1, -1, -1};
+    for (int i = first + tid; i <= last; i += kSolveThreads) {
+#pragma unroll
+        for (int jj = 0; jj < kNQ - 1; ++jj) {
+            const int pk = (int)b.colp[(size_t)(jj >> 1) * b.Spad + i], d = (jj & 1) ? (pk >> 16) : ((pk << 16) >> 16), cls = win_class(jj);
+            if (d != 0) { l[cls] = min(l[cls], i + d); h[cls] = max(h[cls], i + d); }
+        }
+    }
+#pragma unroll
+    for (int c = 0; c < 3; ++c) { if (h[c] >= 0) { atomicMin(&lo[c], l[c]); atomicMax(&hi[c], h[c]); } }
+    __syncthreads();
+    if (tid < 3) { const bool any = hi[tid] >= lo[tid]; tab[lb * kWinSlots + 2 * tid] = any ? lo[tid] : 0; tab[lb * kWinSlots + 2 * tid + 1] = any ? hi[tid] : -1; }
+    if (tid >= 6 && tid < kWinSlots) tab[lb * kWinSlots + tid] = 0;
+}
+void launch_solve_window_table(const Band& b, int row0, int row1, int G, int rows_per_wg, int* tab, hipStream_t s) {
+    hipLaunchKernelGGL(k_solve_window_table, dim3(G), dim3(kSolveThreads), 0, s, b, row0, row1, rows_per_wg, tab);
+}
+int cgp_window_batch() { return kWinBatch * kSolveThreads; }
+constexpr size_t kLdsPerWorkgroup = 160 * 1024;
+template <int R> static bool cgp_window_fits_r(size_t win_bytes, size_t* cap) {
+    const void* fn = (const void*)k_cgp_solve<R, false, true, true>;
+    hipFuncAttributes fa;
+    if (hipFuncGetAttributes(&fa, fn) != hipSuccess) return false;
+    const size_t fixed = cgp_solve_lds(R) + fa.sharedSizeBytes;
+    *cap = fixed < kLdsPerWorkgroup ? kLdsPerWorkgroup - fixed : 0;
+    if (win_bytes > *cap) return false;
+    static int granted = -1;
+    if (granted < 0) granted = hipFuncSetAttribute(fn, hipFuncAttributeMaxDynamicSharedMemorySize, (int)(cgp_solve_lds(R) + *cap)) == hipSuccess ? 1 : 0;
+    if (!granted) return false;
+    int n = 0;
+    return hipOccupancyMaxActiveBlocksPerMultiprocessor(&n, k_cgp_solve<R, false, true, true>, kSolveThreads, cgp_solve_lds(R) + win_bytes) == hipSuccess && n >= 1;
+}
+bool cgp_window_fits(int rows_per_wg, size_t win_bytes, size_t* cap) {
+    const int rows = (rows_per_wg + kSolveThreads - 1) / kSolveThreads;
+    *cap = 0;
+    return rows == 1 ? cgp_window_fits_r<1>(win_bytes, cap) : rows == 2 ? cgp_window_fits_r<2>(win_bytes, cap) : rows == 3 ? cgp_window_fits_r<3>(win_bytes, cap) : false;
+}
 template <int R> static int cgf_solve_prepare_both() {
     const int classic = std::min(std::min(cgf_solve_prepare<R, false, false>(), cgf_solve_prepare<R, true, false>()), cgf_solve_prepare<R, true, true>());
     if (R > kCgpMaxRows) return classic;
@@ -1065,6 +1191,9 @@
     if (a.pcg_asm && a.pcg_pipe && R <= kCgpMaxRows) {
         if (xr && xr->n_ranks > 1 && a.pcg_pipe == 3) hipLaunchKernelGGL((k_cgp_solve<R, true, true>), dim3(G), dim3(kSolveThreads), cgp_solve_lds(R), s, a, fs, gran, rows_per_wg, kmax, mb, mb_key, force_passes, *xr);
         else if (xr && xr->n_ranks > 1) hipLaunchKernelGGL((k_cgp_solve<R, true>), dim3(G), dim3(kSolveThreads), cgp_solve_lds(R), s, a, fs, gran, rows_per_wg, kmax, mb, mb_key, force_passes, *xr);
+        else if (a.pcg_pipe >= 2 && R <= 3 && a.pcg_win && a.pcg_win_G == G && a.pcg_win_rows == rows_per_wg && !((a.pcg_xcd_local >> 3) & 7)) {
+            if constexpr (R <= 3) hipLaunchKernelGGL((k_cgp_solve<R, false, true, true>), dim3(G), dim3(kSolveThreads), cgp_solve_lds(R) + (size_t)a.pcg_win_bytes, s, a, fs, gran, rows_per_wg, kmax, mb, mb_key, force_passes, none);
+        }
         else if (a.pcg_pipe >= 2) { hipLaunchKernelGGL((k_cgp_solve<R, false, true>), dim3(G), dim3(kSolveThreads), cgp_solve_lds(R), s, a, fs, gran, rows_per_wg, kmax, mb, mb_key, force_passes, none); }
         else hipLaunchKernelGGL((k_cgp_solve<R, false>), dim3(G), dim3(kSolveThreads), cgp_solve_lds(R), s, a, fs, gran, rows_per_wg, kmax, mb, mb_key, force_passes, none);
         return;
```

After: 2845. 2.2% lower.
